# kongzhecn/OMG

Hardware: NVIDIA H100
Metric: 1024^2 images/sec @30 steps, 2 concepts (higher is better)
Workload: dtype f16

## Files before the change

### omg_b200/csrc/attn_relpos.cu

```cuda
#include <cuda_fp16.h>

#include <algorithm>
#include <math.h>
#include <string.h>

#include "../../include/omg_b200.h"
#include "host_common.h"
#include "ptx.cuh"
#include "wgmma.cuh"

namespace omg {

constexpr int RP_BQ = 128;
constexpr int RP_BKV = 64;
constexpr int RP_TROWS = 128;
constexpr int RP_STAGES = 3;
constexpr int RP_THREADS = 256;
constexpr float RP_LOG2E = 1.4426950408889634f;

template <int D>
struct RpLayout {
    static constexpr bool X = D > 64;
    static constexpr int Q64 = RP_BQ * 128;
    static constexpr int Q_BYTES = Q64 + (X ? RP_BQ * 32 : 0);
    static constexpr int K64 = RP_BKV * 128, K16 = RP_BKV * 32;
    static constexpr int STAGE = 2 * K64 + (X ? 2 * K16 : 0);
    static constexpr int T64 = RP_TROWS * 128, T16 = RP_TROWS * 32;
    static constexpr int T_BYTES = 2 * T64 + (X ? 2 * T16 : 0);
    static_assert(T_BYTES <= RP_STAGES * STAGE, "tables must fit the K/V ring");
    static constexpr int FIXED = 1024 + Q_BYTES + RP_STAGES * STAGE + 8 * (2 + 2 * RP_STAGES) + 4 * RP_BKV + 4 * RP_BQ;
};

struct alignas(64) RelposParams {
    CUtensorMap q64, q16, kv64, kv16;
    CUtensorMap th64, th16, tw64, tw16;
    const __half* qkv;
    const __half* kb;
    const __half* vb;
    __half* out;
    long long bs, out_bs;
    int ld, out_ld, out_col0;
    int q_col0, k_col0, v_col0;
    int H, W, Wh, Ww;
    int nwx, ntiles, byq, byk, nkb;
    int sh_stride, sw_stride;
    int has_pad;
    float scale_log2;
};

static inline int rp_bias_stride(int S) {
    int s = (S + 7) / 8 * 8;
    return s % 16 == 0 ? s + 8 : s;
}

template <int D>
__global__ void __launch_bounds__(RP_THREADS, 1) attn_relpos_kernel(const __grid_constant__ RelposParams p) {
    using Lt = RpLayout<D>;
    constexpr bool X = Lt::X;
    extern __shared__ uint8_t smem_raw[];
    uint8_t* smem = reinterpret_cast<uint8_t*>((reinterpret_cast<uintptr_t>(smem_raw) + 1023) & ~uintptr_t(1023));
    uint8_t* q_smem = smem;
    uint8_t* kv_smem = q_smem + Lt::Q_BYTES;
    uint64_t* q_full = reinterpret_cast<uint64_t*>(kv_smem + RP_STAGES * Lt::STAGE);
    uint64_t* t_full = q_full + 1;
    uint64_t* kv_full = q_full + 2;
    uint64_t* kv_empty = kv_full + RP_STAGES;
    int* kmap = reinterpret_cast<int*>(kv_empty + RP_STAGES);
    float* qkb = reinterpret_cast<float*>(kmap + RP_BKV);
    float* bias_h = qkb + RP_BQ;
    float* bias_w = bias_h + RP_BQ * p.sh_stride;

    const int warp = threadIdx.x >> 5, lane = threadIdx.x & 31;
    const int tile = blockIdx.x % p.ntiles, grp = blockIdx.x / p.ntiles;
    const int y0 = (grp / p.nwx) * p.Wh, x0 = (grp % p.nwx) * p.Ww;
    const int head = blockIdx.y, img = blockIdx.z;
    const int nq_box = p.Ww * p.byq, nk_box = p.Ww * p.byk;
    const int qc = p.q_col0 + head * D, kc = p.k_col0 + head * D, vc = p.v_col0 + head * D;
    const int qy_base = tile * p.byq;

    for (int i = threadIdx.x; i < (RP_BQ - nq_box) * 8; i += RP_THREADS)
        reinterpret_cast<uint4*>(q_smem + nq_box * 128)[i] = make_uint4(0, 0, 0, 0);
    if (X)
        for (int i = threadIdx.x; i < (RP_BQ - nq_box) * 2; i += RP_THREADS)
            reinterpret_cast<uint4*>(q_smem + Lt::Q64 + nq_box * 32)[i] = make_uint4(0, 0, 0, 0);
    if (threadIdx.x == 0) {
        tma_prefetch_desc(&p.q64);
        tma_prefetch_desc(&p.kv64);
        mbar_init(q_full, 1);
        mbar_init(t_full, 1);
        for (int i = 0; i < RP_STAGES; ++i) {
            mbar_init(&kv_full[i], 1);
            mbar_init(&kv_empty[i], 2);
        }
        fence_barrier_init();
    }
    if (threadIdx.x < RP_BKV) {
        const int kr = threadIdx.x;
        kmap[kr] = kr < nk_box ? ((kr / p.Ww) << 8) | (kr % p.Ww) : -1;
    }
    fence_proxy_async_smem();
    __syncthreads();
    griddep_launch_dependents();
    griddep_wait();
    if (threadIdx.x == 0) {
        mbar_arrive_expect_tx(q_full, nq_box * D * 2);
        tma_load_4d(q_smem, &p.q64, q_full, qc, x0, y0 + qy_base, img);
        if (X) tma_load_4d(q_smem + Lt::Q64, &p.q16, q_full, qc + 64, x0, y0 + qy_base, img);
        mbar_arrive_expect_tx(t_full, 2 * RP_TROWS * D * 2);
        tma_load_2d(kv_smem, &p.th64, t_full, 0, 0);
        tma_load_2d(kv_smem + Lt::T64, &p.tw64, t_full, 0, 0);
        if (X) {
            tma_load_2d(kv_smem + 2 * Lt::T64, &p.th16, t_full, 64, 0);
            tma_load_2d(kv_smem + 2 * Lt::T64 + Lt::T16, &p.tw16, t_full, 64, 0);
        }
    }
    if (p.has_pad && threadIdx.x < RP_BQ) {
        const int r = threadIdx.x;
        const int gy = y0 + qy_base + r / p.Ww, gx = x0 + r % p.Ww;
        float acc = 0.f;
        if (r < nq_box && gy < p.H && gx < p.W) {
            const __half* q = p.qkv + img * p.bs + (long long)(gy * p.W + gx) * p.ld + qc;
            const __half* kb = p.kb + head * D;
#pragma unroll 8
            for (int d = 0; d < D; ++d) acc = fmaf(__half2float(q[d]), __half2float(kb[d]), acc);
        }
        qkb[r] = acc * p.scale_log2;
    }

    const int wg = warp >> 2, wi = warp & 3;
    const int g = lane >> 2, c = lane & 3;
    const int row0 = wg * 64 + wi * 16 + g;
    const uint32_t q_addr = smem_u32(q_smem) + wg * (64 * 128);
    const uint32_t q16_addr = smem_u32(q_smem + Lt::Q64) + wg * (64 * 32);
    mbar_wait(q_full, 0);
    mbar_wait(t_full, 0);
#pragma unroll 1
    for (int t = 0; t < 2; ++t) {
        const int S = t ? p.Ww : p.Wh;
        float* bias = t ? bias_w : bias_h;
        const int stride = t ? p.sw_stride : p.sh_stride;
        const uint32_t t_addr = smem_u32(kv_smem) + t * Lt::T64;
        const uint32_t t16_addr = smem_u32(kv_smem) + 2 * Lt::T64 + t * Lt::T16;
        int qpos[2];
#pragma unroll
        for (int hh = 0; hh < 2; ++hh) {
            const int r = row0 + 8 * hh;
            qpos[hh] = t ? r % p.Ww : min(qy_base + r / p.Ww, p.Wh - 1);
        }
#pragma unroll 1
        for (int ch = 0; ch * 64 < 2 * S - 1; ++ch) {
            float acc[32];
#pragma unroll
            for (int i = 0; i < 32; ++i) acc[i] = 0.f;
            wgmma_fence();
#pragma unroll
            for (int k = 0; k < 4; ++k)
                wgmma_ss_n64(acc, gmma_desc_sw128(q_addr + k * 32, 1024, 16),
                             gmma_desc_sw128(t_addr + ch * 8192 + k * 32, 1024, 16), 1u);
            if (X) wgmma_ss_n64(acc, gmma_desc_sw32(q16_addr), gmma_desc_sw32(t16_addr + ch * 2048), 1u);
            wgmma_commit();
            wgmma_wait<0>();
            reg_fence(acc);
#pragma unroll
            for (int J = 0; J < 8; ++J)
#pragma unroll
                for (int hh = 0; hh < 2; ++hh)
#pragma unroll
                    for (int e = 0; e < 2; ++e) {
                        const int k = qpos[hh] + S - 1 - (ch * 64 + 8 * J + 2 * c + e);
                        if (k >= 0 && k < S) bias[(row0 + 8 * hh) * stride + k] = acc[4 * J + 2 * hh + e] * RP_LOG2E;
                    }
        }
    }
    __syncthreads();
    for (int st = 0; st < RP_STAGES; ++st) {
        uint8_t* sd = kv_smem + st * Lt::STAGE;
        for (int i = threadIdx.x; i < (RP_BKV - nk_box) * 8; i += RP_THREADS) {
            reinterpret_cast<uint4*>(sd + nk_box * 128)[i] = make_uint4(0, 0, 0, 0);
            reinterpret_cast<uint4*>(sd + Lt::K64 + nk_box * 128)[i] = make_uint4(0, 0, 0, 0);
        }
        if (X)
            for (int i = threadIdx.x; i < (RP_BKV - nk_box) * 2; i += RP_THREADS) {
                reinterpret_cast<uint4*>(sd + 2 * Lt::K64 + nk_box * 32)[i] = make_uint4(0, 0, 0, 0);
                reinterpret_cast<uint4*>(sd + 2 * Lt::K64 + Lt::K16 + nk_box * 32)[i] = make_uint4(0, 0, 0, 0);
            }
    }
    fence_proxy_async_smem();
    __syncthreads();

    auto load_kv = [&](int jb) {
        const int st = jb % RP_STAGES;
        mbar_wait(&kv_empty[st], ((jb / RP_STAGES) & 1) ^ 1);
        uint8_t* sd = kv_smem + st * Lt::STAGE;
        const int y = y0 + jb * p.byk;
        mbar_arrive_expect_tx(&kv_full[st], 2 * nk_box * D * 2);
        tma_load_4d(sd, &p.kv64, &kv_full[st], kc, x0, y, img);
        tma_load_4d(sd + Lt::K64, &p.kv64, &kv_full[st], vc, x0, y, img);
        if (X) {
            tma_load_4d(sd + 2 * Lt::K64, &p.kv16, &kv_full[st], kc + 64, x0, y, img);
            tma_load_4d(sd + 2 * Lt::K64 + Lt::K16, &p.kv16, &kv_full[st], vc + 64, x0, y, img);
        }
    };
    if (threadIdx.x == 0)
        for (int jb = 0; jb < RP_STAGES && jb < p.nkb; ++jb) load_kv(jb);

    const float* bh[2] = {bias_h + row0 * p.sh_stride, bias_h + (row0 + 8) * p.sh_stride};
    const float* bw[2] = {bias_w + row0 * p.sw_stride, bias_w + (row0 + 8) * p.sw_stride};
    const float qk[2] = {p.has_pad ? qkb[row0] : 0.f, p.has_pad ? qkb[row0 + 8] : 0.f};
    float o[32], o16[8];
#pragma unroll
    for (int i = 0; i < 32; ++i) o[i] = 0.f;
#pragma unroll
    for (int i = 0; i < 8; ++i) o16[i] = 0.f;
    float m[2] = {-INFINITY, -INFINITY}, l[2] = {0.f, 0.f}, lp[2] = {0.f, 0.f};
    for (int j = 0; j < p.nkb; ++j) {
        const int st = j % RP_STAGES;
        mbar_wait(&kv_full[st], (j / RP_STAGES) & 1);
        const uint32_t k_addr = smem_u32(kv_smem + st * Lt::STAGE);
        float s[32];
#pragma unroll
        for (int i = 0; i < 32; ++i) s[i] = 0.f;
        wgmma_fence();
#pragma unroll
        for (int k = 0; k < 4; ++k)
            wgmma_ss_n64(s, gmma_desc_sw128(q_addr + k * 32, 1024, 16), gmma_desc_sw128(k_addr + k * 32, 1024, 16), 1u);
        if (X) wgmma_ss_n64(s, gmma_desc_sw32(q16_addr), gmma_desc_sw32(k_addr + 2 * Lt::K64), 1u);
        wgmma_commit();
        if (threadIdx.x == 0 && j >= 1 && j - 1 + RP_STAGES < p.nkb) load_kv(j - 1 + RP_STAGES);
        __syncwarp();
        wgmma_wait<0>();
        reg_fence(s);
        uint32_t padbits = 0;
#pragma unroll
        for (int J = 0; J < 8; ++J)
#pragma unroll
            for (int e = 0; e < 2; ++e) {
                const int km = kmap[8 * J + 2 * c + e];
                const int ky = j * p.byk + (km >> 8), kx = km & 255;
                const bool valid = km >= 0 && ky < p.Wh;
                const bool pad = valid && (y0 + ky >= p.H || x0 + kx >= p.W);
                padbits |= (uint32_t)pad << (2 * J + e);
#pragma unroll
                for (int hh = 0; hh < 2; ++hh) {
                    float& v = s[4 * J + 2 * hh + e];
                    v = valid ? fmaf(v, p.scale_log2, bh[hh][ky] + bw[hh][kx] + (pad ? qk[hh] : 0.f)) : -INFINITY;
                }
            }
        float mx[2] = {-INFINITY, -INFINITY};
#pragma unroll
        for (int J = 0; J < 8; ++J)
#pragma unroll
            for (int hh = 0; hh < 2; ++hh) mx[hh] = fmaxf(mx[hh], fmaxf(s[4 * J + 2 * hh], s[4 * J + 2 * hh + 1]));
        float corr[2];
#pragma unroll
        for (int hh = 0; hh < 2; ++hh) {
            mx[hh] = fmaxf(mx[hh], __shfl_xor_sync(0xffffffffu, mx[hh], 1));
            mx[hh] = fmaxf(mx[hh], __shfl_xor_sync(0xffffffffu, mx[hh], 2));
            const float m_new = fmaxf(m[hh], mx[hh]);
            corr[hh] = fast_exp2(m[hh] - m_new);
            m[hh] = m_new;
            l[hh] *= corr[hh];
            lp[hh] *= corr[hh];
        }
#pragma unroll
        for (int J = 0; J < 8; ++J)
#pragma unroll
            for (int hh = 0; hh < 2; ++hh) {
                o[4 * J + 2 * hh] *= corr[hh];
                o[4 * J + 2 * hh + 1] *= corr[hh];
            }
#pragma unroll
        for (int J = 0; J < 2; ++J)
#pragma unroll
            for (int hh = 0; hh < 2; ++hh) {
                o16[4 * J + 2 * hh] *= corr[hh];
                o16[4 * J + 2 * hh + 1] *= corr[hh];
            }
        uint32_t pa[4][4];
#pragma unroll
        for (int kk = 0; kk < 4; ++kk)
#pragma unroll
            for (int t = 0; t < 4; ++t) {
                const int hh = t & 1, J = 2 * kk + (t >> 1), i0 = 4 * J + 2 * hh;
                const float p0 = fast_exp2(s[i0] - m[hh]);
                const float p1 = fast_exp2(s[i0 + 1] - m[hh]);
                l[hh] += p0 + p1;
                if (padbits >> (2 * J) & 1u) lp[hh] += p0;
                if (padbits >> (2 * J + 1) & 1u) lp[hh] += p1;
                pa[kk][t] = pack_half2(p0, p1);
            }
        const uint32_t v_addr = k_addr + Lt::K64;
        const uint32_t v16_addr = k_addr + 2 * Lt::K64 + Lt::K16;
        wgmma_fence();
#pragma unroll
        for (int kk = 0; kk < 4; ++kk) {
            wgmma_rs_n64_tb(o, pa[kk], gmma_desc_sw128(v_addr + kk * 2048, 1024, 1024), 1u);
            if (X) wgmma_rs_n16_tb(o16, pa[kk], gmma_desc_sw32(v16_addr + kk * 512), 1u);
        }
        wgmma_commit();
        wgmma_wait<0>();
        reg_fence(o);
        if constexpr (X) reg_fence(o16);
        if ((threadIdx.x & 127) == 0) mbar_arrive(&kv_empty[st]);
    }

#pragma unroll
    for (int hh = 0; hh < 2; ++hh) {
        l[hh] += __shfl_xor_sync(0xffffffffu, l[hh], 1);
        l[hh] += __shfl_xor_sync(0xffffffffu, l[hh], 2);
        lp[hh] += __shfl_xor_sync(0xffffffffu, lp[hh], 1);
        lp[hh] += __shfl_xor_sync(0xffffffffu, lp[hh], 2);
        const int r = row0 + 8 * hh;
        const int qy = qy_base + r / p.Ww, qx = r % p.Ww;
        const int gy = y0 + qy, gx = x0 + qx;
        if (r >= nq_box || qy >= p.Wh || gy >= p.H || gx >= p.W) continue;
        const float inv = 1.f / l[hh];
        __half* op = p.out + img * p.out_bs + (long long)(gy * p.W + gx) * p.out_ld + p.out_col0 + head * D + 2 * c;
        const __half* vb = p.has_pad ? p.vb + head * D + 2 * c : nullptr;
#pragma unroll
        for (int J = 0; J < 8; ++J) {
            float v0 = o[4 * J + 2 * hh], v1 = o[4 * J + 2 * hh + 1];
            if (vb) {
                v0 = fmaf(lp[hh], __half2float(vb[8 * J]), v0);
                v1 = fmaf(lp[hh], __half2float(vb[8 * J + 1]), v1);
            }
            *reinterpret_cast<__half2*>(op + 8 * J) = __floats2half2_rn(v0 * inv, v1 * inv);
        }
        if (X)
#pragma unroll
            for (int J = 0; J < 2; ++J) {
                float v0 = o16[4 * J + 2 * hh], v1 = o16[4 * J + 2 * hh + 1];
                if (vb) {
                    v0 = fmaf(lp[hh], __half2float(vb[64 + 8 * J]), v0);
                    v1 = fmaf(lp[hh], __half2float(vb[64 + 8 * J + 1]), v1);
                }
                *reinterpret_cast<__half2*>(op + 64 + 8 * J) = __floats2half2_rn(v0 * inv, v1 * inv);
            }
    }
}

static size_t rp_smem_bytes(int D, int Wh, int Ww) {
    const size_t fixed = D > 64 ? RpLayout<80>::FIXED : RpLayout<64>::FIXED;
    return fixed + (size_t)4 * RP_BQ * (rp_bias_stride(Wh) + rp_bias_stride(Ww));
}

template <int D>
static int launch_relpos(RelposParams& p, dim3 grid, size_t smem, cudaStream_t stream) {
    static bool configured = false;
    if (!configured) {
        OMG_CUDA(cudaFuncSetAttribute(attn_relpos_kernel<D>, cudaFuncAttributeMaxDynamicSharedMemorySize,
                                      (int)rp_smem_bytes(D, 64, 64)));
        configured = true;
    }
    OMG_CUDA(launch_pdl(attn_relpos_kernel<D>, grid, dim3(RP_THREADS), smem, stream, p));
    return check_launch(D > 64 ? "attn_relpos_kernel<80>" : "attn_relpos_kernel<64>");
}

}

using namespace omg;

static int relpos_impl(const omg_attn_relpos_desc* d, void* stream_) {
    static const char* who = "omg_attention_relpos";
    OMG_CHECK(d != nullptr, "%s: null descriptor", who);
    OMG_CHECK(d->head_dim == 64 || d->head_dim == 80, "%s: head_dim %d unsupported (SAM ViT-B/L use 64, ViT-H 80)", who,
              d->head_dim);
    OMG_CHECK(d->B >= 1 && d->H >= 1 && d->W >= 1 && d->heads >= 1, "%s: empty problem", who);
    OMG_CHECK(d->window >= 0 && d->window <= 64, "%s: window %d out of range [0, 64]", who, d->window);
    OMG_CHECK(d->window > 0 || (d->H <= 64 && d->W <= 64), "%s: global attention over a %d x %d grid (at most 64 x 64)",
              who, d->H, d->W);
    const int Wh = d->window ? d->window : d->H, Ww = d->window ? d->window : d->W;
    OMG_CHECK(d->rel_h_len == 2 * Wh - 1, "%s: rel_pos_h has %d rows, expected 2 * %d - 1 = %d (no interpolation)", who,
              d->rel_h_len, Wh, 2 * Wh - 1);
    OMG_CHECK(d->rel_w_len == 2 * Ww - 1, "%s: rel_pos_w has %d rows, expected 2 * %d - 1 = %d (no interpolation)", who,
              d->rel_w_len, Ww, 2 * Ww - 1);
    OMG_CHECK(d->qkv && d->out && d->rel_pos_h && d->rel_pos_w, "%s: null pointer", who);
    const bool pad = d->window > 0 && (d->H % d->window || d->W % d->window);
    OMG_CHECK(!pad || (d->k_bias && d->v_bias),
              "%s: a %d x %d grid in windows of %d is padded: k_bias and v_bias (the padded tokens' key and value) are "
              "required", who, d->H, d->W, d->window);
    OMG_CHECK(((uintptr_t)d->qkv & 15) == 0 && d->ld % 8 == 0 && d->bs % 8 == 0,
              "%s: qkv rows must be 16 B aligned (pointer, ld, bs)", who);
    OMG_CHECK(((uintptr_t)d->rel_pos_h & 15) == 0 && ((uintptr_t)d->rel_pos_w & 15) == 0,
              "%s: rel-pos tables must be 16 B aligned", who);
    OMG_CHECK(((uintptr_t)d->out & 15) == 0 && d->out_ld % 8 == 0 && d->out_col0 % 8 == 0 && d->out_bs % 8 == 0,
              "%s: output must be 16 B aligned per row", who);
    if (check_head_windows(who, d->heads, d->head_dim, {d->q_col0, d->k_col0, d->v_col0, d->out_col0},
                           {d->ld, d->ld, d->ld, d->out_ld}))
        return 1;

    const int D = d->head_dim;
    RelposParams p;
    memset(&p, 0, sizeof(p));
    const int byq = std::min(RP_BQ / Ww, Wh), byk = std::min(RP_BKV / Ww, Wh);
    const uint64_t dims[4] = {(uint64_t)d->ld, (uint64_t)d->W, (uint64_t)d->H, (uint64_t)d->B};
    const uint64_t strides[4] = {1, (uint64_t)d->ld, (uint64_t)d->ld * d->W, (uint64_t)d->bs};
    const uint32_t bq64[4] = {64, (uint32_t)Ww, (uint32_t)byq, 1}, bq16[4] = {16, (uint32_t)Ww, (uint32_t)byq, 1};
    const uint32_t bk64[4] = {64, (uint32_t)Ww, (uint32_t)byk, 1}, bk16[4] = {16, (uint32_t)Ww, (uint32_t)byk, 1};
    const auto F16 = CU_TENSOR_MAP_DATA_TYPE_FLOAT16;
    if (make_tmap(&p.q64, F16, d->qkv, 4, dims, strides, bq64, CU_TENSOR_MAP_SWIZZLE_128B)) return 1;
    if (make_tmap(&p.kv64, F16, d->qkv, 4, dims, strides, bk64, CU_TENSOR_MAP_SWIZZLE_128B)) return 1;
    const uint64_t th_dims[2] = {(uint64_t)D, (uint64_t)d->rel_h_len}, tw_dims[2] = {(uint64_t)D, (uint64_t)d->rel_w_len};
    const uint64_t t_str[2] = {1, (uint64_t)D};
    const uint32_t bt64[2] = {64, RP_TROWS}, bt16[2] = {16, RP_TROWS};
    if (make_tmap(&p.th64, F16, d->rel_pos_h, 2, th_dims, t_str, bt64, CU_TENSOR_MAP_SWIZZLE_128B)) return 1;
    if (make_tmap(&p.tw64, F16, d->rel_pos_w, 2, tw_dims, t_str, bt64, CU_TENSOR_MAP_SWIZZLE_128B)) return 1;
    if (D > 64) {
        if (make_tmap(&p.q16, F16, d->qkv, 4, dims, strides, bq16, CU_TENSOR_MAP_SWIZZLE_32B)) return 1;
        if (make_tmap(&p.kv16, F16, d->qkv, 4, dims, strides, bk16, CU_TENSOR_MAP_SWIZZLE_32B)) return 1;
        if (make_tmap(&p.th16, F16, d->rel_pos_h, 2, th_dims, t_str, bt16, CU_TENSOR_MAP_SWIZZLE_32B)) return 1;
        if (make_tmap(&p.tw16, F16, d->rel_pos_w, 2, tw_dims, t_str, bt16, CU_TENSOR_MAP_SWIZZLE_32B)) return 1;
    }
    p.qkv = static_cast<const __half*>(d->qkv);
    p.kb = static_cast<const __half*>(d->k_bias);
    p.vb = static_cast<const __half*>(d->v_bias);
    p.out = static_cast<__half*>(d->out);
    p.bs = d->bs;
    p.out_bs = d->out_bs;
    p.ld = d->ld;
    p.out_ld = d->out_ld;
    p.out_col0 = d->out_col0;
    p.q_col0 = d->q_col0;
    p.k_col0 = d->k_col0;
    p.v_col0 = d->v_col0;
    p.H = d->H;
    p.W = d->W;
    p.Wh = Wh;
    p.Ww = Ww;
    p.nwx = (d->W + Ww - 1) / Ww;
    p.byq = byq;
    p.byk = byk;
    p.ntiles = (Wh + byq - 1) / byq;
    p.nkb = (Wh + byk - 1) / byk;
    p.sh_stride = rp_bias_stride(Wh);
    p.sw_stride = rp_bias_stride(Ww);
    p.has_pad = pad;
    p.scale_log2 = d->scale * RP_LOG2E;
    const int nwy = (d->H + Wh - 1) / Wh;
    const dim3 grid(nwy * p.nwx * p.ntiles, d->heads, d->B);
    const size_t smem = rp_smem_bytes(D, Wh, Ww);
    cudaStream_t stream = reinterpret_cast<cudaStream_t>(stream_);
    return D > 64 ? launch_relpos<80>(p, grid, smem, stream) : launch_relpos<64>(p, grid, smem, stream);
}

extern "C" int omg_attention_relpos(const omg_attn_relpos_desc* d, void* stream_) {
    const int rc = relpos_impl(d, stream_);
    if (rc == 0 && ::omg::plan_recording()) {
        const omg_attn_relpos_desc c = *d;
        ::omg::plan_note([c](void* s) { return relpos_impl(&c, s); });
    }
    return rc;
}
```

### omg_b200/csrc/attn_tc.cu

```cuda
#include <cuda_fp16.h>

#include <algorithm>
#include <math.h>
#include <stdlib.h>
#include <string.h>

#include "../../include/omg_b200.h"
#include "host_common.h"
#include "ptx.cuh"
#include "wgmma.cuh"

namespace omg {

constexpr int ATT_BQ = 128;
constexpr int ATT_BKV = 64;
constexpr int ATT_D = 64;
constexpr int ATT_Q_BYTES = ATT_BQ * ATT_D * 2;
constexpr int ATT_K_BYTES = ATT_BKV * ATT_D * 2;
constexpr int ATT_KV_STAGES = 4;
constexpr int ATT_THREADS = 256;
constexpr int ATT_SMEM = 1024 + ATT_Q_BYTES + ATT_KV_STAGES * 2 * ATT_K_BYTES + 256;

struct alignas(64) AttnParams {
    CUtensorMap q_map, k_map, v_map;
    __half* out;
    int out_ld;
    long long out_bs;
    int n_q, n_kv, heads;
    int q_col0, k_col0, v_col0, out_col0;
    int n_items;
    int out_b[OMG_ATTN_MAX_ITEMS], q_b[OMG_ATTN_MAX_ITEMS], k_b[OMG_ATTN_MAX_ITEMS], v_b[OMG_ATTN_MAX_ITEMS];
    float scale_log2;
    float out_weight;
    int accumulate;
    int causal;
};

__global__ void __launch_bounds__(ATT_THREADS, 2) attn_tc_kernel(const __grid_constant__ AttnParams p) {
    extern __shared__ uint8_t smem_raw[];
    uint8_t* smem = reinterpret_cast<uint8_t*>((reinterpret_cast<uintptr_t>(smem_raw) + 1023) & ~uintptr_t(1023));
    uint8_t* q_smem = smem;
    uint8_t* kv_smem = q_smem + ATT_Q_BYTES;
    uint64_t* q_full = reinterpret_cast<uint64_t*>(kv_smem + ATT_KV_STAGES * 2 * ATT_K_BYTES);
    uint64_t* kv_full = q_full + 1;
    uint64_t* kv_empty = kv_full + ATT_KV_STAGES;

    const int warp = threadIdx.x >> 5;
    const int lane = threadIdx.x & 31;
    const int slab = blockIdx.x, head = blockIdx.y, item = blockIdx.z;
    const int nkv = (p.n_kv + ATT_BKV - 1) / ATT_BKV;

    const int kb = p.k_b[item], vb = p.v_b[item];
    auto load_kv = [&](int jb) {
        const int st = jb % ATT_KV_STAGES;
        mbar_wait(&kv_empty[st], ((jb / ATT_KV_STAGES) & 1) ^ 1);
        uint8_t* kd = kv_smem + st * 2 * ATT_K_BYTES;
        mbar_arrive_expect_tx(&kv_full[st], 2 * ATT_K_BYTES);
        tma_load_3d(kd, &p.k_map, &kv_full[st], p.k_col0 + head * ATT_D, jb * ATT_BKV, kb);
        tma_load_3d(kd + ATT_K_BYTES, &p.v_map, &kv_full[st], p.v_col0 + head * ATT_D, jb * ATT_BKV, vb);
    };
    if (threadIdx.x == 0) {
        tma_prefetch_desc(&p.q_map);
        tma_prefetch_desc(&p.k_map);
        tma_prefetch_desc(&p.v_map);
        mbar_init(q_full, 1);
        for (int i = 0; i < ATT_KV_STAGES; ++i) {
            mbar_init(&kv_full[i], 1);
            mbar_init(&kv_empty[i], 2);
        }
        fence_barrier_init();
    }
    __syncthreads();
    griddep_launch_dependents();
    griddep_wait();
    if (threadIdx.x == 0) {
        mbar_arrive_expect_tx(q_full, ATT_Q_BYTES);
        tma_load_3d(q_smem, &p.q_map, q_full, p.q_col0 + head * ATT_D, slab * ATT_BQ, p.q_b[item]);
        for (int jb = 0; jb < ATT_KV_STAGES && jb < nkv; ++jb) load_kv(jb);
    }

    const int wg = warp >> 2, wi = warp & 3;
    const int g = lane >> 2, c = lane & 3;
    const int qrow0 = slab * ATT_BQ + wg * 64 + wi * 16 + g;
    const uint32_t q_addr = smem_u32(q_smem) + wg * (64 * 128);
    float o[32];
#pragma unroll
    for (int i = 0; i < 32; ++i) o[i] = 0.f;
    float m[2] = {-INFINITY, -INFINITY}, l[2] = {0.f, 0.f};
    mbar_wait(q_full, 0);
    for (int j = 0; j < nkv; ++j) {
        const int st = j % ATT_KV_STAGES;
        mbar_wait(&kv_full[st], (j / ATT_KV_STAGES) & 1);
        const uint32_t k_addr = smem_u32(kv_smem + st * 2 * ATT_K_BYTES);
        float s[32];
#pragma unroll
        for (int i = 0; i < 32; ++i) s[i] = 0.f;
        wgmma_fence();
#pragma unroll
        for (int k = 0; k < ATT_D / 16; ++k)
            wgmma_ss_n64(s, gmma_desc_sw128(q_addr + k * 32, 1024, 16), gmma_desc_sw128(k_addr + k * 32, 1024, 16), 1u);
        wgmma_commit();
        if (threadIdx.x == 0 && j >= 1 && j - 1 + ATT_KV_STAGES < nkv) load_kv(j - 1 + ATT_KV_STAGES);
        __syncwarp();
        wgmma_wait<0>();
        reg_fence(s);
        const int key0 = j * ATT_BKV + 2 * c;
        if ((j + 1) * ATT_BKV > p.n_kv || p.causal) {
#pragma unroll
            for (int J = 0; J < 8; ++J)
#pragma unroll
                for (int h = 0; h < 2; ++h)
#pragma unroll
                    for (int e = 0; e < 2; ++e) {
                        const int key = key0 + 8 * J + e;
                        if (key >= p.n_kv || (p.causal && key > qrow0 + 8 * h)) s[4 * J + 2 * h + e] = -INFINITY;
                    }
        }
        float mx[2] = {-INFINITY, -INFINITY};
#pragma unroll
        for (int J = 0; J < 8; ++J)
#pragma unroll
            for (int h = 0; h < 2; ++h) mx[h] = fmaxf(mx[h], fmaxf(s[4 * J + 2 * h], s[4 * J + 2 * h + 1]));
        float corr[2];
#pragma unroll
        for (int h = 0; h < 2; ++h) {
            mx[h] = fmaxf(mx[h], __shfl_xor_sync(0xffffffffu, mx[h], 1));
            mx[h] = fmaxf(mx[h], __shfl_xor_sync(0xffffffffu, mx[h], 2));
            const float m_new = fmaxf(m[h], mx[h] * p.scale_log2);
            corr[h] = fast_exp2(m[h] - m_new);
            m[h] = m_new;
            l[h] *= corr[h];
        }
#pragma unroll
        for (int J = 0; J < 8; ++J)
#pragma unroll
            for (int h = 0; h < 2; ++h) {
                o[4 * J + 2 * h] *= corr[h];
                o[4 * J + 2 * h + 1] *= corr[h];
            }
        uint32_t pa[4][4];
#pragma unroll
        for (int kk = 0; kk < 4; ++kk)
#pragma unroll
            for (int t = 0; t < 4; ++t) {
                const int h = t & 1, i0 = 8 * kk + 4 * (t >> 1) + 2 * h;
                const float p0 = fast_exp2(fmaf(s[i0], p.scale_log2, -m[h]));
                const float p1 = fast_exp2(fmaf(s[i0 + 1], p.scale_log2, -m[h]));
                l[h] += p0 + p1;
                pa[kk][t] = pack_half2(p0, p1);
            }
        const uint32_t v_addr = k_addr + ATT_K_BYTES;
        wgmma_fence();
#pragma unroll
        for (int kk = 0; kk < 4; ++kk)
            wgmma_rs_n64_tb(o, pa[kk], gmma_desc_sw128(v_addr + kk * 2048, 1024, 1024), 1u);
        wgmma_commit();
        wgmma_wait<0>();
        reg_fence(o);
        if ((threadIdx.x & 127) == 0) mbar_arrive(&kv_empty[st]);
    }

#pragma unroll
    for (int h = 0; h < 2; ++h) {
        l[h] += __shfl_xor_sync(0xffffffffu, l[h], 1);
        l[h] += __shfl_xor_sync(0xffffffffu, l[h], 2);
        const int qrow = qrow0 + 8 * h;
        if (qrow < p.n_q) {
            const float inv = p.out_weight / l[h];
            __half* op = p.out + (long long)p.out_b[item] * p.out_bs + (long long)qrow * p.out_ld + p.out_col0 +
                         head * ATT_D + 2 * c;
#pragma unroll
            for (int J = 0; J < 8; ++J) {
                float v0 = o[4 * J + 2 * h] * inv, v1 = o[4 * J + 2 * h + 1] * inv;
                __half2* dst = reinterpret_cast<__half2*>(op + 8 * J);
                if (p.accumulate) {
                    const float2 f = __half22float2(*dst);
                    v0 += f.x;
                    v1 += f.y;
                }
                *dst = __floats2half2_rn(v0, v1);
            }
        }
    }
}

static int make_attn_map(CUtensorMap* m, const void* ptr, int cols, int ld, int tokens, long long bs, int nb,
                         uint32_t box_rows) {
    const uint64_t dims[3] = {(uint64_t)cols, (uint64_t)tokens, (uint64_t)nb};
    const uint64_t strides[3] = {1, (uint64_t)ld, (uint64_t)bs};
    const uint32_t box[3] = {64, box_rows, 1};
    return make_tmap(m, CU_TENSOR_MAP_DATA_TYPE_FLOAT16, ptr, 3, dims, strides, box, CU_TENSOR_MAP_SWIZZLE_128B);
}

}

using namespace omg;

static int attention_impl(const omg_attn_desc* d, void* stream_) {
    cudaStream_t stream = reinterpret_cast<cudaStream_t>(stream_);
    OMG_CHECK(d != nullptr, "omg_attention: null descriptor");
    OMG_CHECK(d->head_dim == 64, "omg_attention: head_dim %d unsupported (SDXL uses 64)", d->head_dim);
    OMG_CHECK(d->n_items >= 1 && d->n_items <= OMG_ATTN_MAX_ITEMS, "omg_attention: n_items=%d out of range",
              d->n_items);
    OMG_CHECK(d->n_q >= 1 && d->n_kv >= 1 && d->heads >= 1, "omg_attention: empty problem");
    OMG_CHECK(d->q && d->k && d->v && d->out, "omg_attention: null pointer");
    OMG_CHECK(d->out_ld % 8 == 0 && d->out_col0 % 8 == 0 && d->out_bs % 8 == 0,
              "omg_attention: output must be 16 B aligned per row");
    if (check_head_windows("omg_attention", d->heads, d->head_dim, {d->q_col0, d->k_col0, d->v_col0, d->out_col0},
                           {d->q_ld, d->k_ld, d->v_ld, d->out_ld}))
        return 1;
    OMG_CHECK(!d->causal || (d->n_kv <= 128 && d->n_q <= 128), "omg_attention: causal masking is available for sequences of <= 128 tokens");
    static bool configured = false;
    if (!configured) {
        OMG_CUDA(cudaFuncSetAttribute(attn_tc_kernel, cudaFuncAttributeMaxDynamicSharedMemorySize, ATT_SMEM));
        configured = true;
    }
    AttnParams p;
    memset(&p, 0, sizeof(p));
    int max_qb = 0, max_kb = 0, max_vb = 0;
    for (int i = 0; i < d->n_items; ++i) {
        p.out_b[i] = d->out_b[i];
        p.q_b[i] = d->q_b[i];
        p.k_b[i] = d->k_b[i];
        p.v_b[i] = d->v_b[i];
        max_qb = d->q_b[i] > max_qb ? d->q_b[i] : max_qb;
        max_kb = d->k_b[i] > max_kb ? d->k_b[i] : max_kb;
        max_vb = d->v_b[i] > max_vb ? d->v_b[i] : max_vb;
        OMG_CHECK(d->out_b[i] >= 0 && d->q_b[i] >= 0 && d->k_b[i] >= 0 && d->v_b[i] >= 0,
                  "omg_attention: negative batch index in item %d", i);
    }
    const int cols = d->heads * 64;
    if (make_attn_map(&p.q_map, d->q, d->q_col0 + cols, d->q_ld, d->n_q, d->q_bs, max_qb + 1, ATT_BQ)) return 1;
    if (make_attn_map(&p.k_map, d->k, d->k_col0 + cols, d->k_ld, d->n_kv, d->k_bs, max_kb + 1, ATT_BKV)) return 1;
    if (make_attn_map(&p.v_map, d->v, d->v_col0 + cols, d->v_ld, d->n_kv, d->v_bs, max_vb + 1, ATT_BKV)) return 1;
    p.out = static_cast<__half*>(d->out);
    p.out_ld = d->out_ld;
    p.out_bs = d->out_bs;
    p.n_q = d->n_q;
    p.n_kv = d->n_kv;
    p.heads = d->heads;
    p.q_col0 = d->q_col0;
    p.k_col0 = d->k_col0;
    p.v_col0 = d->v_col0;
    p.out_col0 = d->out_col0;
    p.n_items = d->n_items;
    p.scale_log2 = d->scale * 1.4426950408889634f;
    p.out_weight = d->out_weight;
    p.accumulate = d->accumulate;
    p.causal = d->causal;
    dim3 grid((d->n_q + ATT_BQ - 1) / ATT_BQ, d->heads, d->n_items);
    OMG_CUDA(launch_pdl(attn_tc_kernel, grid, dim3(ATT_THREADS), ATT_SMEM, stream, p));
    return check_launch("attn_tc_kernel");
}

extern "C" int omg_attention(const omg_attn_desc* d, void* stream_) {
    const int rc = attention_impl(d, stream_);
    if (rc == 0 && ::omg::plan_recording()) {
        const omg_attn_desc c = *d;
        ::omg::plan_note([c](void* s) { return attention_impl(&c, s); });
    }
    return rc;
}
```

### omg_b200/csrc/gemm_tc.cu

```cuda
#include <cuda_fp16.h>
#include <stdlib.h>
#include <string.h>

#include <algorithm>
#include <type_traits>

#include "../../include/omg_b200.h"
#include "elem.cuh"
#include "host_common.h"
#include "ptx.cuh"
#include "wgmma.cuh"

namespace omg {

constexpr int BM = 128;
constexpr int BK = 64;
constexpr int GEMM_THREADS = 384;

struct SegDev {
    int a_map, dx, dy, a_c0, k_blocks, b_k0, b_map;
};

struct alignas(64) GemmParams {
    CUtensorMap a_maps[OMG_MAX_A];
    CUtensorMap b_maps[2];
    SegDev segs[OMG_MAX_SEGS];
    int n_segs;
    int m_tiles, n_tiles;
    int tw, th, tiles_w, tiles_h;
    int img_w, img_h, img_b;
    int N, N_out;
    void* out;
    long long out_sw, out_sh, out_sb;
    const void* bias;
    const void* rowvec;
    int rowvec_ld;
    const void* residual;
    int residual_ld;
    int act_silu;
    float* stats_out;
    const float* stats_in;
    int stats_parts;
    long long stats_rows;
    float ln_inv_dim, ln_eps;
    const float* col_c1;
    const float* col_c2;
    int n_col_groups;
    long long col_group_end[8];
    int w_group_rows;
    const float* residual_f32;
    long long residual_f32_ld;
    float* out_f32;
    long long out_f32_ld;
    float4* col_stats;
    int cs_rb0, cs_rb_total;
};

template <int BN, int MT, bool CS>
struct GemmCfg {
    static constexpr int WN = BN > 256 ? BN / 2 : BN;
    static constexpr int NW = BN / WN;
    static constexpr int ACC = MT * BN / 2;
    static constexpr int A_BYTES = MT * BM * BK * 2;
    static constexpr int B_BYTES = BN * BK * 2;
    static constexpr int STAGE_BYTES = A_BYTES + B_BYTES;
    static constexpr int VEC_BYTES = 2 * MT * BN * 4;
    static constexpr int CS_BYTES = CS ? 8 * MT * BN * 8 : 0;
    static constexpr int BARS_BYTES = 256;
    static constexpr int BUDGET = 227 * 1024 - 1024  - VEC_BYTES - CS_BYTES - BARS_BYTES;
    static constexpr int STAGES_RAW = BUDGET / STAGE_BYTES;
    static constexpr int STAGES = STAGES_RAW > 8 ? 8 : STAGES_RAW;
    static constexpr int SMEM_BYTES = 1024 + STAGES * STAGE_BYTES + VEC_BYTES + CS_BYTES + BARS_BYTES;
    static_assert(STAGES >= 2, "shared memory budget");
};

__device__ __forceinline__ float gelu_exact(float x) { return 0.5f * x * (1.0f + erff(x * 0.70710678118654752f)); }

template <typename T, int WN>
__device__ __forceinline__ void wgmma_ss(float* d, uint64_t da, uint64_t db) {
    if constexpr (std::is_same_v<T, __nv_bfloat16>) {
        if constexpr (WN == 64) wgmma_ss_n64_bf16(*reinterpret_cast<float(*)[32]>(d), da, db, 1u);
        else if constexpr (WN == 128) wgmma_ss_n128_bf16(*reinterpret_cast<float(*)[64]>(d), da, db, 1u);
        else if constexpr (WN == 160) wgmma_ss_n160_bf16(*reinterpret_cast<float(*)[80]>(d), da, db, 1u);
        else wgmma_ss_n256_bf16(*reinterpret_cast<float(*)[128]>(d), da, db, 1u);
    } else {
        if constexpr (WN == 64) wgmma_ss_n64(*reinterpret_cast<float(*)[32]>(d), da, db, 1u);
        else if constexpr (WN == 128) wgmma_ss_n128(*reinterpret_cast<float(*)[64]>(d), da, db, 1u);
        else if constexpr (WN == 160) wgmma_ss_n160(*reinterpret_cast<float(*)[80]>(d), da, db, 1u);
        else wgmma_ss_n256(*reinterpret_cast<float(*)[128]>(d), da, db, 1u);
    }
}

template <typename T, int BN, int EPI, int MT, int FEAT>
__global__ void __launch_bounds__(GEMM_THREADS, 1) gemm_tc_kernel(const __grid_constant__ GemmParams p) {
    using T2 = pair_t<T>;
    constexpr bool kStats = FEAT >= 1, kExtra = FEAT >= 2;
    static_assert(EPI != OMG_EPI_GEGLU || (BN <= 256 && MT == 1), "GEGLU runs on single 128-row tiles");
    using Cfg = GemmCfg<BN, MT, kStats>;
    constexpr int STAGES = Cfg::STAGES;
    constexpr int NJ = BN / 8;
    extern __shared__ __align__(1024) uint8_t smem_raw[];
    uint8_t* smem = reinterpret_cast<uint8_t*>((reinterpret_cast<uintptr_t>(smem_raw) + 1023) & ~uintptr_t(1023));
    float* s_bias = reinterpret_cast<float*>(smem + STAGES * Cfg::STAGE_BYTES);
    float* s_c1 = s_bias + MT * BN;
    float4* s_cs = reinterpret_cast<float4*>(s_c1 + MT * BN);
    uint64_t* full_bar = reinterpret_cast<uint64_t*>(reinterpret_cast<uint8_t*>(s_cs) + Cfg::CS_BYTES);
    uint64_t* empty_bar = full_bar + STAGES;

    const int warp = threadIdx.x >> 5;
    const int lane = threadIdx.x & 31;
    const int total_tiles = ((p.m_tiles + MT - 1) / MT) * p.n_tiles;
    const int tiles_per_img = p.tiles_w * p.tiles_h;

    if (warp == 8 && lane == 0) {
        for (int i = 0; i < OMG_MAX_A; ++i) tma_prefetch_desc(&p.a_maps[i]);
        tma_prefetch_desc(&p.b_maps[0]);
        tma_prefetch_desc(&p.b_maps[1]);
        for (int i = 0; i < STAGES; ++i) {
            mbar_init(&full_bar[i], 1);
            mbar_init(&empty_bar[i], 2);
        }
        fence_barrier_init();
    }
    __syncthreads();
    griddep_launch_dependents();
    griddep_wait();

    if (warp >= 8) {
        asm volatile("setmaxnreg.dec.sync.aligned.u32 40;");
        if (warp == 8 && lane == 0) {
            int stage = 0;
            uint32_t phase = 0;
            for (int tile = blockIdx.x; tile < total_tiles; tile += gridDim.x) {
                const int m_tile = (tile / p.n_tiles) * MT, n_tile = tile % p.n_tiles;
                const int b = m_tile / tiles_per_img;
                const int rem = m_tile % tiles_per_img;
                const int h0 = (rem / p.tiles_w) * p.th, w0 = (rem % p.tiles_w) * p.tw;
                const int b1 = (m_tile + 1) / tiles_per_img, rem1 = (m_tile + 1) % tiles_per_img;
                const int h1 = (rem1 / p.tiles_w) * p.th, w1 = (rem1 % p.tiles_w) * p.tw;
                int n0 = n_tile * BN;
                if (p.w_group_rows > 0) {
                    const long long tile_pix0 = ((long long)b * p.img_h + h0) * p.img_w + w0;
                    for (int g2 = 0; g2 + 1 < p.n_col_groups; ++g2)
                        if (tile_pix0 >= p.col_group_end[g2]) n0 += p.w_group_rows;
                }
                for (int s = 0; s < p.n_segs; ++s) {
                    const SegDev sg = p.segs[s];
                    for (int kb = 0; kb < sg.k_blocks; ++kb) {
                        mbar_wait(&empty_bar[stage], phase ^ 1);
                        uint8_t* a_dst = smem + stage * Cfg::STAGE_BYTES;
                        uint8_t* b_dst = a_dst + Cfg::A_BYTES;
                        mbar_arrive_expect_tx(&full_bar[stage], Cfg::STAGE_BYTES);
                        tma_load_4d(a_dst, &p.a_maps[sg.a_map], &full_bar[stage], sg.a_c0 + kb * BK, w0 + sg.dx, h0 + sg.dy, b);
                        if constexpr (MT == 2)
                            tma_load_4d(a_dst + BM * BK * 2, &p.a_maps[sg.a_map], &full_bar[stage], sg.a_c0 + kb * BK,
                                        w1 + sg.dx, h1 + sg.dy, b1);
#pragma unroll
                        for (int nw = 0; nw < Cfg::NW; ++nw)
                            tma_load_2d(b_dst + nw * Cfg::WN * BK * 2, &p.b_maps[sg.b_map], &full_bar[stage],
                                        sg.b_k0 + kb * BK, n0 + nw * Cfg::WN);
                        if (++stage == STAGES) {
                            stage = 0;
                            phase ^= 1;
                        }
                    }
                }
            }
        }
        return;
    }

    asm volatile("setmaxnreg.inc.sync.aligned.u32 232;");
    const int wg = warp >> 2;
    const int wi = warp & 3;
    const int g = lane >> 2, c = lane & 3;
    const int ctid = threadIdx.x;
    int stage = 0;
    uint32_t phase = 0;
    float acc[Cfg::ACC];

    for (int tile = blockIdx.x; tile < total_tiles; tile += gridDim.x) {
        const int unit_m = (tile / p.n_tiles) * MT, n_tile = tile % p.n_tiles;
        const int n0 = n_tile * BN;
        const bool ln = p.stats_in != nullptr;

        named_bar_sync(1, 256);
        for (int sub = 0; sub < MT; ++sub) {
            const int mt = unit_m + sub;
            const int b = mt / tiles_per_img, rem = mt % tiles_per_img;
            size_t cg = 0;
            if (ln && p.n_col_groups > 1) {
                const long long tile_pix0 = ((long long)b * p.img_h + (rem / p.tiles_w) * p.th) * p.img_w + (rem % p.tiles_w) * p.tw;
                for (int g2 = 0; g2 + 1 < p.n_col_groups; ++g2)
                    if (tile_pix0 >= p.col_group_end[g2]) cg = g2 + 1;
                cg *= (size_t)p.N;
            }
            for (int j = ctid; j < BN; j += 256) {
                float v = 0.f, c1 = 0.f;
                const int n = n0 + j;
                if (n < p.N) {
                    if (ln) {
                        v = p.col_c2[cg + n];
                        c1 = p.col_c1[cg + n];
                    } else {
                        if (p.bias) v += to_f32(static_cast<const T*>(p.bias)[n]);
                        if (p.rowvec && b < p.img_b) v += to_f32(static_cast<const T*>(p.rowvec)[(size_t)b * p.rowvec_ld + n]);
                    }
                }
                s_bias[sub * BN + j] = v;
                s_c1[sub * BN + j] = c1;
            }
        }
        named_bar_sync(1, 256);

#pragma unroll
        for (int i = 0; i < Cfg::ACC; ++i) acc[i] = 0.f;
        int prev_stage = -1;
        for (int s = 0; s < p.n_segs; ++s) {
            const int kbs = p.segs[s].k_blocks;
            for (int kb = 0; kb < kbs; ++kb) {
                mbar_wait(&full_bar[stage], phase);
                const uint32_t a_addr = smem_u32(smem + stage * Cfg::STAGE_BYTES) + (uint32_t)(wg * MT) * (64 * BK * 2);
                const uint32_t b_addr = smem_u32(smem + stage * Cfg::STAGE_BYTES + Cfg::A_BYTES);
                wgmma_fence();
#pragma unroll
                for (int k = 0; k < BK / 16; ++k) {
#pragma unroll
                    for (int i = 0; i < MT; ++i) {
                        const uint64_t a_desc = gmma_desc_sw128(a_addr + i * (64 * BK * 2) + k * 32, 1024, 16);
#pragma unroll
                        for (int nw = 0; nw < Cfg::NW; ++nw) {
                            const uint64_t b_desc = gmma_desc_sw128(b_addr + nw * (Cfg::WN * BK * 2) + k * 32, 1024, 16);
                            wgmma_ss<T, Cfg::WN>(acc + i * (BN / 2) + nw * (Cfg::WN / 2), a_desc, b_desc);
                        }
                    }
                }
                wgmma_commit();
                wgmma_wait<1>();
                if (prev_stage >= 0 && (ctid & 127) == 0) mbar_arrive(&empty_bar[prev_stage]);
                prev_stage = stage;
                if (++stage == STAGES) {
                    stage = 0;
                    phase ^= 1;
                }
            }
        }
        wgmma_wait<0>();
        reg_fence(acc);
        if ((ctid & 127) == 0) mbar_arrive(&empty_bar[prev_stage]);

#pragma unroll
        for (int i = 0; i < MT; ++i) {
            const int blk = wg * MT + i;
            const int sub = blk >> 1;
            const int m_tile = unit_m + sub;
            const int b = m_tile / tiles_per_img;
            const int rem = m_tile % tiles_per_img;
            const int h0 = (rem / p.tiles_w) * p.th, w0 = (rem % p.tiles_w) * p.tw;
            const float* sb = s_bias + sub * BN;
            const float* sc = s_c1 + sub * BN;
            float* a = acc + i * (BN / 2);
            float row_sum[2] = {0.f, 0.f}, row_sq[2] = {0.f, 0.f};
            bool valid[2];
            size_t pix[2];
            T* orow[2];
            float ln_a[2] = {1.f, 1.f}, ln_k[2] = {0.f, 0.f};
#pragma unroll
            for (int h = 0; h < 2; ++h) {
                const int et = (blk & 1) * 64 + wi * 16 + g + 8 * h;
                const int ph = h0 + et / p.tw, pw = w0 + et % p.tw;
                valid[h] = (ph < p.img_h) && (pw < p.img_w) && (b < p.img_b);
                pix[h] = ((size_t)b * p.img_h + ph) * p.img_w + pw;
                orow[h] = static_cast<T*>(p.out) + (long long)b * p.out_sb + (long long)ph * p.out_sh + (long long)pw * p.out_sw;
                if (ln && valid[h]) {
                    float sa = 0.f, sq = 0.f;
                    for (int t = 0; t < p.stats_parts; ++t) {
                        const float2 st = __ldg(reinterpret_cast<const float2*>(p.stats_in) + (size_t)t * p.stats_rows + pix[h]);
                        sa += st.x;
                        sq += st.y;
                    }
                    const float mu = sa * p.ln_inv_dim;
                    ln_a[h] = rsqrtf(fmaxf(sq * p.ln_inv_dim - mu * mu, 0.f) + p.ln_eps);
                    ln_k[h] = -ln_a[h] * mu;
                }
            }
            float4* cs_slot = s_cs + (size_t)(blk * 4 + wi) * (BN / 2);
#pragma unroll
            for (int J = 0; J < NJ; ++J) {
                const int col = 8 * J + 2 * c;
                const int n = n0 + col;
                float x[2][2];
#pragma unroll
                for (int h = 0; h < 2; ++h)
#pragma unroll
                    for (int e = 0; e < 2; ++e) {
                        const float v = a[4 * J + 2 * h + e];
                        x[h][e] = ln ? fmaf(ln_a[h], v, fmaf(ln_k[h], sc[col + e], sb[col + e])) : v + sb[col + e];
                    }
                if constexpr (EPI == OMG_EPI_GEGLU) {
#pragma unroll
                    for (int h = 0; h < 2; ++h) {
                        const float o = x[h][0] * gelu_exact(x[h][1]);
                        const float o_nb = __shfl_down_sync(0xffffffffu, o, 1);
                        if ((c & 1) == 0 && valid[h] && n < p.N)
                            *reinterpret_cast<T2*>(orow[h] + (n >> 1)) = from_f32x2<T>(o, o_nb);
                    }
                } else {
                    if constexpr (kExtra) {
#pragma unroll
                        for (int h = 0; h < 2; ++h)
#pragma unroll
                            for (int e = 0; e < 2; ++e) {
                                float v = x[h][e];
                                if (p.act_silu == 1) {
                                    v = v / (1.0f + __expf(-v));
                                } else if (p.act_silu == 2) {
                                    v = v / (1.0f + __expf(-1.702f * v));
                                } else if (p.act_silu == 3) {
                                    v = gelu_exact(v);
                                } else if (p.act_silu == 4) {
                                    const float u = 0.7978845608028654f * fmaf(0.044715f * v * v, v, v);
                                    v = 0.5f * v * (2.0f - __fdividef(2.0f, 1.0f + __expf(2.0f * u)));
                                } else if (p.act_silu == 5) {
                                    v = fmaxf(v, 0.f);
                                }
                                x[h][e] = v;
                            }
                    }
                    float4 cs = make_float4(0.f, 0.f, 0.f, 0.f);
#pragma unroll
                    for (int h = 0; h < 2; ++h) {
                        const bool ok = valid[h] && n < p.N;
                        if (ok && p.residual != nullptr) {
                            const float2 r = to_f32x2(*reinterpret_cast<const T2*>(static_cast<const T*>(p.residual) + pix[h] * (size_t)p.residual_ld + n));
                            x[h][0] += r.x;
                            x[h][1] += r.y;
                        }
                        if constexpr (kExtra) {
                            if (ok && p.residual_f32 != nullptr) {
                                const float2 r = *reinterpret_cast<const float2*>(p.residual_f32 + pix[h] * (size_t)p.residual_f32_ld + n);
                                x[h][0] += r.x;
                                x[h][1] += r.y;
                            }
                            if (ok && p.out_f32 != nullptr)
                                *reinterpret_cast<float2*>(p.out_f32 + pix[h] * (size_t)p.out_f32_ld + n) = make_float2(x[h][0], x[h][1]);
                        }
                        if (ok) {
                            row_sum[h] += x[h][0] + x[h][1];
                            row_sq[h] = fmaf(x[h][0], x[h][0], fmaf(x[h][1], x[h][1], row_sq[h]));
                        }
                        const T2 o = from_f32x2<T>(x[h][0], x[h][1]);
                        if (ok) *reinterpret_cast<T2*>(orow[h] + n) = o;
                        if constexpr (kStats) {
                            const float2 f = valid[h] ? to_f32x2(o) : make_float2(0.f, 0.f);
                            cs.x += f.x;
                            cs.y = fmaf(f.x, f.x, cs.y);
                            cs.z += f.y;
                            cs.w = fmaf(f.y, f.y, cs.w);
                        }
                    }
                    if constexpr (kStats) {
                        if (p.col_stats != nullptr) {
#pragma unroll
                            for (int off = 4; off < 32; off <<= 1) {
                                cs.x += __shfl_xor_sync(0xffffffffu, cs.x, off);
                                cs.y += __shfl_xor_sync(0xffffffffu, cs.y, off);
                                cs.z += __shfl_xor_sync(0xffffffffu, cs.z, off);
                                cs.w += __shfl_xor_sync(0xffffffffu, cs.w, off);
                            }
                            if (g == 0) cs_slot[4 * J + c] = cs;
                        }
                    }
                }
            }
            if constexpr (EPI != OMG_EPI_GEGLU) {
                if (p.stats_out != nullptr) {
                    float2* so = reinterpret_cast<float2*>(p.stats_out);
                    constexpr int PLANES = BN > 256 ? 4 : 2;
#pragma unroll
                    for (int h = 0; h < 2; ++h) {
                        float s = row_sum[h], q = row_sq[h];
                        s += __shfl_xor_sync(0xffffffffu, s, 1);
                        q += __shfl_xor_sync(0xffffffffu, q, 1);
                        s += __shfl_xor_sync(0xffffffffu, s, 2);
                        q += __shfl_xor_sync(0xffffffffu, q, 2);
                        if (c == 0 && valid[h]) {
                            so[(size_t)(n_tile * PLANES) * p.stats_rows + pix[h]] = make_float2(s, q);
                            for (int t = 1; t < PLANES; ++t) so[(size_t)(n_tile * PLANES + t) * p.stats_rows + pix[h]] = make_float2(0.f, 0.f);
                        }
                    }
                }
            }
            if constexpr (EPI != OMG_EPI_GEGLU && kStats) {
                if (p.col_stats != nullptr) {
                    named_bar_sync(2 + wg * 2 + (wi >> 1), 64);
                    const int q = (blk & 1) * 2 + (wi >> 1);
                    const float4* s0 = s_cs + (size_t)(blk * 4 + (wi & 2)) * (BN / 2);
                    const float4* s1 = s0 + BN / 2;
                    if (b < p.img_b) {
                        const size_t rb = (size_t)b * p.cs_rb_total + p.cs_rb0 + (size_t)rem * 4 + q;
                        for (int cp = (wi & 1) * 32 + lane; cp < BN / 2; cp += 64) {
                            const int col = n0 + 2 * cp;
                            if (col < p.N) {
                                const float4 u = s0[cp], w = s1[cp];
                                p.col_stats[(rb * p.N + col) >> 1] = make_float4(u.x + w.x, u.y + w.y, u.z + w.z, u.w + w.w);
                            }
                        }
                    }
                }
            }
        }
    }
}

static int view_to_tmap(CUtensorMap* m, const omg_view4& v, CUtensorMapDataType dt, uint32_t box_c, uint32_t box_w,
                        uint32_t box_h, CUtensorMapSwizzle sw) {
    const uint64_t dims[4] = {(uint64_t)v.C, (uint64_t)v.W, (uint64_t)v.H, (uint64_t)v.B};
    const uint64_t strides[4] = {1, (uint64_t)v.sw, (uint64_t)v.sh, (uint64_t)v.sb};
    const uint32_t box[4] = {box_c, box_w, box_h, 1};
    return make_tmap(m, dt, v.ptr, 4, dims, strides, box, sw);
}

template <typename T, int BN, int EPI, int MT, int FEAT>
static int launch_gemm_f(const GemmParams& p, cudaStream_t stream) {
    using Cfg = GemmCfg<BN, MT, (FEAT >= 1)>;
    static bool configured = false;
    static int num_sms = 0;
    if (!configured) {
        OMG_CUDA(cudaFuncSetAttribute(gemm_tc_kernel<T, BN, EPI, MT, FEAT>, cudaFuncAttributeMaxDynamicSharedMemorySize,
                                      Cfg::SMEM_BYTES));
        int dev = 0;
        OMG_CUDA(cudaGetDevice(&dev));
        OMG_CUDA(cudaDeviceGetAttribute(&num_sms, cudaDevAttrMultiProcessorCount, dev));
        configured = true;
    }
    const int units = ((p.m_tiles + MT - 1) / MT) * p.n_tiles;
    const int grid = std::min(units, num_sms);
    OMG_CUDA(launch_pdl(gemm_tc_kernel<T, BN, EPI, MT, FEAT>, dim3(grid), dim3(GEMM_THREADS), Cfg::SMEM_BYTES, stream, p));
    return check_launch("gemm_tc_kernel");
}

template <int BN, int EPI, int MT = 1>
static int launch_gemm(const GemmParams& p, cudaStream_t stream) {
    if constexpr (EPI == OMG_EPI_GEGLU) {
        return launch_gemm_f<__half, BN, EPI, MT, 0>(p, stream);
    } else {
        if (p.act_silu != 0 || p.residual_f32 != nullptr || p.out_f32 != nullptr) return launch_gemm_f<__half, BN, EPI, MT, 2>(p, stream);
        if (p.col_stats != nullptr) return launch_gemm_f<__half, BN, EPI, MT, 1>(p, stream);
        return launch_gemm_f<__half, BN, EPI, MT, 0>(p, stream);
    }
}

constexpr int PLAN_SMS = 132;
constexpr double TILE_OVERHEAD = 48.0;
static double tile_time(long tiles, double cols) {
    return (double)((tiles + PLAN_SMS - 1) / PLAN_SMS) * (cols + TILE_OVERHEAD);
}

static bool use_tall_tiles(long m_tiles, long n_tiles, long k_blocks) {
    if (m_tiles < 2 || k_blocks < 16) return false;
    return tile_time(((m_tiles + 1) / 2) * n_tiles, 320.0) < tile_time(m_tiles * n_tiles, 160.0);
}

constexpr long K_PLAN_LONG = 1000;
static int pick_block_n(int N, int epilogue, long m_tiles, long k_plan, long k_blocks, bool* prefer_tall) {
    if (prefer_tall) *prefer_tall = false;
    if (epilogue == OMG_EPI_GEGLU) return 256;
    const int cands[5] = {256, 160, 128, 64, 160};
    int best = 256;
    double best_t = 1e30;
    for (int i = 0; i < 5; ++i) {
        const bool tall = i == 4;
        if (tall && (k_plan < 16 || m_tiles < 2)) continue;
        const long nt = (N + cands[i] - 1) / cands[i];
        const long mt = tall ? (m_tiles + 1) / 2 : m_tiles;
        const double t = tile_time(nt * mt, tall ? 2.0 * cands[i] : cands[i]);
        if (t < best_t - 1e-9) {
            best_t = t;
            best = cands[i];
            if (prefer_tall) *prefer_tall = tall && k_blocks >= 16;
        }
    }
    return best;
}

}

using namespace omg;

extern "C" int omg_gemm_plan(int N, int epilogue, int W, int H, int B, int* block_n, int* n_tiles) {
    OMG_CHECK(N >= 8 && W >= 1 && H >= 1 && B >= 1, "omg_gemm_plan: bad arguments");
    int tw = 128;
    while (tw / 2 >= W && tw > 1) tw /= 2;
    const int th = 128 / tw;
    const long m_tiles = (long)((W + tw - 1) / tw) * ((H + th - 1) / th) * B;
    const int bn = pick_block_n(N, epilogue, m_tiles, K_PLAN_LONG, 0, nullptr);
    if (block_n) *block_n = bn;
    if (n_tiles) *n_tiles = 2 * ((N + bn - 1) / bn);
    return 0;
}

extern "C" int omg_gemm_colstats_blocks(int W, int H) {
    if (W < 1 || H < 1) return 0;
    int tw = 128;
    while (tw / 2 >= W && tw > 1) tw /= 2;
    const int th = 128 / tw;
    return ((W + tw - 1) / tw) * ((H + th - 1) / th) * 4;
}

static int gemm_impl(const omg_gemm_desc* d, void* stream_) {
    cudaStream_t stream = reinterpret_cast<cudaStream_t>(stream_);
    OMG_CHECK(d != nullptr, "omg_gemm: null descriptor");
    OMG_CHECK(d->n_a >= 1 && d->n_a <= OMG_MAX_A, "omg_gemm: n_a=%d out of range", d->n_a);
    OMG_CHECK(d->n_segs >= 1 && d->n_segs <= OMG_MAX_SEGS, "omg_gemm: n_segs=%d out of range", d->n_segs);
    OMG_CHECK(d->w && d->d.ptr, "omg_gemm: null weight/output pointer");
    OMG_CHECK(d->N >= 8 && d->N % 8 == 0, "omg_gemm: N=%d must be a positive multiple of 8", d->N);
    OMG_CHECK(d->Ktot % 8 == 0, "omg_gemm: Ktot=%d must be a multiple of 8", d->Ktot);
    OMG_CHECK(d->dtype == OMG_DTYPE_F16 || d->dtype == OMG_DTYPE_BF16, "omg_gemm: dtype=%d unsupported (0 fp16, 1 bf16)",
              d->dtype);
    const bool bf16 = d->dtype == OMG_DTYPE_BF16;
    if (bf16) {
        OMG_CHECK(d->epilogue == OMG_EPI_NONE, "omg_gemm: bf16 supports only OMG_EPI_NONE (epilogue %d)", d->epilogue);
        OMG_CHECK(!d->rowvec, "omg_gemm: bf16 does not support rowvec");
        OMG_CHECK(!d->w2, "omg_gemm: bf16 does not support a second weight matrix (w2)");
        OMG_CHECK(d->w_group_planes == 0, "omg_gemm: bf16 does not support weight planes");
        OMG_CHECK(!d->row_stats_in, "omg_gemm: bf16 does not support the folded LayerNorm");
        OMG_CHECK(!d->row_stats_out, "omg_gemm: bf16 does not support row statistics");
        OMG_CHECK(!d->col_stats_out, "omg_gemm: bf16 does not support column statistics");
        OMG_CHECK(!d->residual_f32 && !d->out_f32, "omg_gemm: bf16 does not support fp32 twins");
    }
    const CUtensorMapDataType tdt = bf16 ? CU_TENSOR_MAP_DATA_TYPE_BFLOAT16 : CU_TENSOR_MAP_DATA_TYPE_FLOAT16;
    const bool geglu = d->epilogue == OMG_EPI_GEGLU;
    const bool silu = d->epilogue == OMG_EPI_SILU;
    const int act = silu ? 1 : (d->epilogue == OMG_EPI_QUICK_GELU ? 2 : (d->epilogue == OMG_EPI_GELU ? 3 : (d->epilogue == OMG_EPI_GELU_TANH ? 4 :
                    (d->epilogue == OMG_EPI_RELU ? 5 : 0))));
    OMG_CHECK(d->epilogue == OMG_EPI_NONE || geglu || act, "omg_gemm: unknown epilogue %d", d->epilogue);
    const int N_out = geglu ? d->N / 2 : d->N;
    OMG_CHECK(d->d.C == N_out, "omg_gemm: output view has %d channels, expected %d", d->d.C, N_out);
    OMG_CHECK(!geglu || (d->N % 64 == 0 && !d->residual && !d->rowvec),
              "omg_gemm: GEGLU needs N %% 64 == 0 and no residual/rowvec");
    OMG_CHECK(!d->residual || (N_out % 32 == 0 && d->residual_ld % 8 == 0),
              "omg_gemm: residual needs N %% 32 == 0 and ld %% 8 == 0");

    GemmParams p;
    memset(&p, 0, sizeof(p));
    const int W = d->d.W, H = d->d.H, B = d->d.B;
    OMG_CHECK(W >= 1 && H >= 1 && B >= 1, "omg_gemm: empty output grid");
    int tw = 128;
    while (tw / 2 >= W && tw > 1) tw /= 2;
    const int th = 128 / tw;
    p.tw = tw;
    p.th = th;
    p.tiles_w = (W + tw - 1) / tw;
    p.tiles_h = (H + th - 1) / th;
    p.img_w = W;
    p.img_h = H;
    p.img_b = B;
    p.m_tiles = p.tiles_w * p.tiles_h * B;
    p.N = d->N;
    p.N_out = N_out;
    bool prefer_tall = false;
    const long k_blocks_hint = (long)(d->Ktot + (d->w2 ? d->K2tot : 0)) / 64;
    int bn = d->block_n ? d->block_n
                        : pick_block_n(d->N, d->epilogue, p.m_tiles, d->row_stats_out ? K_PLAN_LONG : k_blocks_hint,
                                       k_blocks_hint, &prefer_tall);
    OMG_CHECK(bn == 64 || bn == 128 || bn == 160 || bn == 256 || bn == 320, "omg_gemm: block_n=%d unsupported", bn);
    OMG_CHECK(bn != 320 || (!geglu && d->N % 320 == 0), "omg_gemm: block_n=320 needs N %% 320 == 0 and no GEGLU");
    OMG_CHECK(d->cta_pair == 0 || d->cta_pair == 1 || d->cta_pair == 3, "omg_gemm: cta_pair=%d unsupported (0, 1 or 3)",
              d->cta_pair);
    if (geglu) bn = 256;
    p.n_tiles = (d->N + bn - 1) / bn;
    p.bias = d->bias;
    p.rowvec = d->rowvec;
    p.rowvec_ld = d->rowvec_ld;
    p.residual = d->residual;
    p.residual_ld = d->residual_ld;
    p.act_silu = act;
    p.stats_out = static_cast<float*>(d->row_stats_out);
    p.stats_in = static_cast<const float*>(d->row_stats_in);
    p.stats_parts = d->row_stats_parts;
    p.stats_rows = d->row_stats_stride > 0 ? d->row_stats_stride : (long long)W * H * B;
    p.ln_inv_dim = d->ln_dim > 0 ? 1.0f / (float)d->ln_dim : 0.f;
    p.ln_eps = d->ln_eps;
    p.col_c1 = static_cast<const float*>(d->col_c1);
    p.col_c2 = static_cast<const float*>(d->col_c2);
    p.n_col_groups = d->n_col_groups > 0 ? d->n_col_groups : 1;
    p.w_group_rows = d->w_group_planes > 0 ? d->N : 0;
    OMG_CHECK(d->w_group_planes == 0 || d->w_group_planes == p.n_col_groups, "omg_gemm: w_group_planes must equal n_col_groups");
    OMG_CHECK(p.n_col_groups <= 8, "omg_gemm: at most 8 column-vector row groups");
    OMG_CHECK(d->w_group_planes == 0 || !d->w2, "omg_gemm: weight planes do not extend to the second weight matrix (w2)");
    const long long img_pix = (long long)W * H;
    for (int i = 0; i < 8; ++i) {
        p.col_group_end[i] = d->col_group_end[i];
        if (i + 1 >= p.n_col_groups) continue;
        if (H > 1)
            OMG_CHECK(d->col_group_end[i] % img_pix == 0,
                      "omg_gemm: row-group boundary %lld is inside an image of the %d x %d output grid (boundaries are "
                      "multiples of %lld pixels)", (long long)d->col_group_end[i], W, H, img_pix);
        else
            OMG_CHECK(d->col_group_end[i] % 128 == 0, "omg_gemm: row-group boundary %lld is not a multiple of the 128-row tile",
                      (long long)d->col_group_end[i]);
    }
    OMG_CHECK(!p.stats_in || (p.col_c1 && p.col_c2 && d->ln_dim > 0 && d->row_stats_parts >= 1 && !d->rowvec),
              "omg_gemm: folded LayerNorm needs col_c1, col_c2, ln_dim, row_stats_parts and no rowvec");
    OMG_CHECK(!p.stats_out || !geglu, "omg_gemm: row statistics cannot be emitted by the GEGLU epilogue");
    p.residual_f32 = static_cast<const float*>(d->residual_f32);
    p.residual_f32_ld = d->residual_f32_ld;
    p.out_f32 = static_cast<float*>(d->out_f32);
    p.out_f32_ld = d->out_f32_ld;
    OMG_CHECK((!p.residual_f32 && !p.out_f32) || (!geglu && d->N % 32 == 0 && !(d->residual && d->residual_f32)),
              "omg_gemm: fp32 residual / output twins need a non-GEGLU epilogue, N %% 32 == 0, and replace the fp16 residual");
    OMG_CHECK((!p.residual_f32 || d->residual_f32_ld % 4 == 0) && (!p.out_f32 || d->out_f32_ld % 4 == 0),
              "omg_gemm: fp32 twin row strides must be multiples of 4");
    OMG_CHECK((!p.residual_f32 && !p.out_f32) || (d->d.sw == d->d.C && d->d.sh == (int64_t)d->d.sw * W && d->d.sb == d->d.sh * H),
              "omg_gemm: fp32 twins need a contiguous output view (rows are indexed by pixel)");
    p.col_stats = static_cast<float4*>(d->col_stats_out);
    p.cs_rb0 = d->col_stats_rb0;
    p.cs_rb_total = d->col_stats_rb_total;
    OMG_CHECK(!p.col_stats || (!geglu && d->N % 32 == 0 && d->col_stats_rb0 >= 0 &&
                               d->col_stats_rb0 + p.tiles_w * p.tiles_h * 4 <= d->col_stats_rb_total),
              "omg_gemm: column statistics need a non-GEGLU epilogue, N %% 32 == 0 and rb0 + blocks <= rb_total");
    OMG_CHECK((!p.stats_out && !p.stats_in) || (d->d.sw == d->d.C && d->d.sh == (int64_t)d->d.sw * W && d->d.sb == d->d.sh * H),
              "omg_gemm: row statistics need a contiguous output view");

    for (int i = 0; i < d->n_a; ++i) {
        OMG_CHECK(d->a[i].ptr != nullptr, "omg_gemm: A view %d is null", i);
        if (view_to_tmap(&p.a_maps[i], d->a[i], tdt, BK, tw, th, CU_TENSOR_MAP_SWIZZLE_128B)) return 1;
    }
    for (int i = d->n_a; i < OMG_MAX_A; ++i) p.a_maps[i] = p.a_maps[0];
    {
        const uint64_t planes = d->w_group_planes > 0 ? (uint64_t)d->w_group_planes : 1;
        const uint64_t dims[2] = {(uint64_t)d->Ktot, (uint64_t)d->N * planes};
        const uint64_t strides[2] = {1, (uint64_t)d->Ktot};
        const uint32_t box[2] = {BK, (uint32_t)(bn > 256 ? bn / 2 : bn)};
        if (make_tmap(&p.b_maps[0], tdt, d->w, 2, dims, strides, box, CU_TENSOR_MAP_SWIZZLE_128B)) return 1;
        p.b_maps[1] = p.b_maps[0];
    }
    if (d->w2 != nullptr) {
        OMG_CHECK(d->K2tot >= 8 && d->K2tot % 8 == 0, "omg_gemm: K2tot=%d must be a positive multiple of 8", d->K2tot);
        const uint64_t dims[2] = {(uint64_t)d->K2tot, (uint64_t)d->N};
        const uint64_t strides[2] = {1, (uint64_t)d->K2tot};
        const uint32_t box[2] = {BK, (uint32_t)(bn > 256 ? bn / 2 : bn)};
        if (make_tmap(&p.b_maps[1], tdt, d->w2, 2, dims, strides, box, CU_TENSOR_MAP_SWIZZLE_128B)) return 1;
    }
    OMG_CHECK(d->d.sw % 2 == 0 && d->d.sh % 2 == 0 && d->d.sb % 2 == 0 && (reinterpret_cast<uintptr_t>(d->d.ptr) & 3) == 0,
              "omg_gemm: output view must be 4 B aligned per pixel");
    p.out = const_cast<void*>(d->d.ptr);
    p.out_sw = d->d.sw;
    p.out_sh = d->d.sh;
    p.out_sb = d->d.sb;

    p.n_segs = d->n_segs;
    for (int s = 0; s < d->n_segs; ++s) {
        const omg_seg& sg = d->segs[s];
        OMG_CHECK(sg.a_idx >= 0 && sg.a_idx < d->n_a, "omg_gemm: segment %d references A view %d", s, sg.a_idx);
        OMG_CHECK(sg.k_len > 0 && sg.a_c0 >= 0 && sg.b_k0 >= 0 && sg.a_c0 + sg.k_len <= d->a[sg.a_idx].C,
                  "omg_gemm: segment %d has a bad K range", s);
        OMG_CHECK(sg.b_idx == 0 || (sg.b_idx == 1 && d->w2 != nullptr), "omg_gemm: segment %d has a bad b_idx", s);
        const int ktot_s = sg.b_idx ? d->K2tot : d->Ktot;
        OMG_CHECK(sg.b_k0 + sg.k_len <= ktot_s, "omg_gemm: segment %d exceeds weight K (%d + %d > %d)", s, sg.b_k0,
                  sg.k_len, ktot_s);
        OMG_CHECK(sg.k_len % BK == 0 || sg.a_c0 + sg.k_len == d->a[sg.a_idx].C,
                  "omg_gemm: segment %d: K tail must end at the A view's last channel", s);
        p.segs[s] = SegDev{sg.a_idx, sg.dx, sg.dy, sg.a_c0, (sg.k_len + BK - 1) / BK, sg.b_k0, sg.b_idx};
    }

    long k_blocks = 0;
    for (int i = 0; i < p.n_segs; ++i) k_blocks += p.segs[i].k_blocks;
    bool pair_ok = true;
    for (int i = 0; i + 1 < p.n_col_groups; ++i)
        pair_ok = pair_ok && (H > 1 ? (p.col_group_end[i] / img_pix * p.tiles_w * p.tiles_h) % 2 == 0
                                    : p.col_group_end[i] % 256 == 0);
    const bool tall = bn == 160 && !geglu && pair_ok &&
                      (d->cta_pair == 3 ||
                       (d->cta_pair == 0 && (prefer_tall || use_tall_tiles(p.m_tiles, p.n_tiles, k_blocks))));
    if (bf16) {
        if (tall) return launch_gemm_f<__nv_bfloat16, 160, OMG_EPI_NONE, 2, 0>(p, stream);
        switch (bn) {
            case 64: return launch_gemm_f<__nv_bfloat16, 64, OMG_EPI_NONE, 1, 0>(p, stream);
            case 128: return launch_gemm_f<__nv_bfloat16, 128, OMG_EPI_NONE, 1, 0>(p, stream);
            case 160: return launch_gemm_f<__nv_bfloat16, 160, OMG_EPI_NONE, 1, 0>(p, stream);
            case 320: return launch_gemm_f<__nv_bfloat16, 320, OMG_EPI_NONE, 1, 0>(p, stream);
            default: return launch_gemm_f<__nv_bfloat16, 256, OMG_EPI_NONE, 1, 0>(p, stream);
        }
    }
    if (bn == 320) return launch_gemm<320, OMG_EPI_NONE>(p, stream);
    if (tall) return launch_gemm<160, OMG_EPI_NONE, 2>(p, stream);
    if (geglu) return launch_gemm<256, OMG_EPI_GEGLU>(p, stream);
    switch (bn) {
        case 64: return launch_gemm<64, OMG_EPI_NONE>(p, stream);
        case 128: return launch_gemm<128, OMG_EPI_NONE>(p, stream);
        case 160: return launch_gemm<160, OMG_EPI_NONE>(p, stream);
        default: return launch_gemm<256, OMG_EPI_NONE>(p, stream);
    }
}

extern "C" int omg_gemm(const omg_gemm_desc* d, void* stream_) {
    const int rc = gemm_impl(d, stream_);
    if (rc == 0 && ::omg::plan_recording()) {
        const omg_gemm_desc c = *d;
        ::omg::plan_note([c](void* s) { return gemm_impl(&c, s); });
    }
    return rc;
}
```

### omg_b200/csrc/ptx.cuh

```cuda
#pragma once
#include <cuda.h>
#include <cuda_fp16.h>
#include <cuda_runtime.h>
#include <stdint.h>
#include <stdio.h>

namespace omg {

__device__ __forceinline__ uint32_t smem_u32(const void* p) {
    return static_cast<uint32_t>(__cvta_generic_to_shared(p));
}

__device__ __forceinline__ uint32_t lane_id() { return threadIdx.x & 31; }

__device__ __forceinline__ bool elect_one() {
    uint32_t pred;
    asm volatile(
        "{\n\t.reg .pred p;\n\t"
        "elect.sync _|p, 0xffffffff;\n\t"
        "selp.u32 %0, 1, 0, p;\n\t}\n"
        : "=r"(pred));
    return pred != 0;
}

__device__ __forceinline__ void griddep_launch_dependents() { asm volatile("griddepcontrol.launch_dependents;" ::: "memory"); }
__device__ __forceinline__ void griddep_wait() { asm volatile("griddepcontrol.wait;" ::: "memory"); }

__device__ __forceinline__ void mbar_init(uint64_t* bar, uint32_t count) {
    asm volatile("mbarrier.init.shared::cta.b64 [%0], %1;" ::"r"(smem_u32(bar)), "r"(count));
}
__device__ __forceinline__ void fence_barrier_init() {
    asm volatile("fence.mbarrier_init.release.cluster;" ::: "memory");
}
__device__ __forceinline__ void fence_proxy_async_smem() {
    asm volatile("fence.proxy.async.shared::cta;" ::: "memory");
}
__device__ __forceinline__ void mbar_arrive_expect_tx(uint64_t* bar, uint32_t bytes) {
    asm volatile("mbarrier.arrive.expect_tx.shared::cta.b64 _, [%0], %1;" ::"r"(smem_u32(bar)), "r"(bytes)
                 : "memory");
}
__device__ __forceinline__ void mbar_arrive(uint64_t* bar) {
    asm volatile("mbarrier.arrive.shared::cta.b64 _, [%0];" ::"r"(smem_u32(bar)) : "memory");
}
__device__ __forceinline__ bool mbar_try_wait(uint64_t* bar, uint32_t parity) {
    uint32_t ok;
    asm volatile(
        "{\n\t.reg .pred p;\n\t"
        "mbarrier.try_wait.parity.shared::cta.b64 p, [%1], %2;\n\t"
        "selp.u32 %0, 1, 0, p;\n\t}\n"
        : "=r"(ok)
        : "r"(smem_u32(bar)), "r"(parity)
        : "memory");
    return ok != 0;
}
#ifndef OMG_MBAR_TIMEOUT_CYCLES
#define OMG_MBAR_TIMEOUT_CYCLES (4000000000LL)
#endif
#ifndef OMG_MBAR_SUSPEND_NS
#define OMG_MBAR_SUSPEND_NS 20000
#endif
__device__ __forceinline__ bool mbar_try_wait_long(uint64_t* bar, uint32_t parity) {
    uint32_t ok;
    asm volatile(
        "{\n\t.reg .pred p;\n\t"
        "mbarrier.try_wait.parity.shared::cta.b64 p, [%1], %2, %3;\n\t"
        "selp.u32 %0, 1, 0, p;\n\t}\n"
        : "=r"(ok)
        : "r"(smem_u32(bar)), "r"(parity), "r"((uint32_t)OMG_MBAR_SUSPEND_NS)
        : "memory");
    return ok != 0;
}
__device__ __forceinline__ void mbar_wait(uint64_t* bar, uint32_t parity) {
    if (mbar_try_wait(bar, parity)) return;
    const long long t0 = clock64();
    uint32_t spins = 0;
    while (!mbar_try_wait_long(bar, parity)) {
        if ((++spins & 0x3FF) == 0 && clock64() - t0 > OMG_MBAR_TIMEOUT_CYCLES) {
            printf("omg: mbarrier timeout block=(%d,%d,%d) thread=%d bar=%u parity=%u\n", (int)blockIdx.x,
                   (int)blockIdx.y, (int)blockIdx.z, (int)threadIdx.x, smem_u32(bar), parity);
            __trap();
        }
    }
}

__device__ __forceinline__ float fast_exp2(float x) {
    float y;
    asm("ex2.approx.ftz.f32 %0, %1;" : "=f"(y) : "f"(x));
    return y;
}

__device__ __forceinline__ void tma_prefetch_desc(const CUtensorMap* m) {
    asm volatile("prefetch.tensormap [%0];" ::"l"(reinterpret_cast<uint64_t>(m)) : "memory");
}
__device__ __forceinline__ void tma_load_2d(void* smem_dst, const CUtensorMap* m, uint64_t* bar, int c0, int c1) {
    asm volatile(
        "cp.async.bulk.tensor.2d.shared::cluster.global.mbarrier::complete_tx::bytes [%0], [%1, {%3, %4}], [%2];"
        ::"r"(smem_u32(smem_dst)), "l"(reinterpret_cast<uint64_t>(m)), "r"(smem_u32(bar)), "r"(c0), "r"(c1)
        : "memory");
}
__device__ __forceinline__ void tma_load_3d(void* smem_dst, const CUtensorMap* m, uint64_t* bar, int c0, int c1,
                                            int c2) {
    asm volatile(
        "cp.async.bulk.tensor.3d.shared::cluster.global.mbarrier::complete_tx::bytes [%0], [%1, {%3, %4, %5}], [%2];"
        ::"r"(smem_u32(smem_dst)), "l"(reinterpret_cast<uint64_t>(m)), "r"(smem_u32(bar)), "r"(c0), "r"(c1), "r"(c2)
        : "memory");
}
__device__ __forceinline__ void tma_load_4d(void* smem_dst, const CUtensorMap* m, uint64_t* bar, int c0, int c1,
                                            int c2, int c3) {
    asm volatile(
        "cp.async.bulk.tensor.4d.shared::cluster.global.mbarrier::complete_tx::bytes [%0], [%1, {%3, %4, %5, %6}], "
        "[%2];"
        ::"r"(smem_u32(smem_dst)), "l"(reinterpret_cast<uint64_t>(m)), "r"(smem_u32(bar)), "r"(c0), "r"(c1), "r"(c2),
        "r"(c3)
        : "memory");
}
__device__ __forceinline__ void tma_store_3d(const CUtensorMap* m, const void* smem_src, int c0, int c1, int c2) {
    asm volatile("cp.async.bulk.tensor.3d.global.shared::cta.bulk_group [%0, {%2, %3, %4}], [%1];" ::"l"(
                     reinterpret_cast<uint64_t>(m)),
                 "r"(smem_u32(smem_src)), "r"(c0), "r"(c1), "r"(c2)
                 : "memory");
}
__device__ __forceinline__ void tma_store_4d(const CUtensorMap* m, const void* smem_src, int c0, int c1, int c2,
                                             int c3) {
    asm volatile("cp.async.bulk.tensor.4d.global.shared::cta.bulk_group [%0, {%2, %3, %4, %5}], [%1];" ::"l"(
                     reinterpret_cast<uint64_t>(m)),
                 "r"(smem_u32(smem_src)), "r"(c0), "r"(c1), "r"(c2), "r"(c3)
                 : "memory");
}
__device__ __forceinline__ void tma_store_commit() { asm volatile("cp.async.bulk.commit_group;" ::: "memory"); }
template <int N>
__device__ __forceinline__ void tma_store_wait_read() {
    asm volatile("cp.async.bulk.wait_group.read %0;" ::"n"(N) : "memory");
}
template <int N>
__device__ __forceinline__ void tma_store_wait_all() {
    asm volatile("cp.async.bulk.wait_group %0;" ::"n"(N) : "memory");
}

__device__ __forceinline__ uint64_t gmma_desc_sw128(uint32_t smem_addr, uint32_t sbo_bytes, uint32_t lbo_bytes) {
    uint64_t d = 0;
    d |= static_cast<uint64_t>((smem_addr & 0x3FFFF) >> 4);
    d |= static_cast<uint64_t>((lbo_bytes >> 4) & 0x3FFF) << 16;
    d |= static_cast<uint64_t>((sbo_bytes >> 4) & 0x3FFF) << 32;
    d |= static_cast<uint64_t>(1) << 62;
    return d;
}
__device__ __forceinline__ uint64_t gmma_desc_sw32(uint32_t smem_addr) {
    uint64_t d = 0;
    d |= static_cast<uint64_t>((smem_addr & 0x3FFFF) >> 4);
    d |= static_cast<uint64_t>(256 >> 4) << 16;
    d |= static_cast<uint64_t>(256 >> 4) << 32;
    d |= static_cast<uint64_t>(3) << 62;
    return d;
}
__device__ __forceinline__ void wgmma_fence() { asm volatile("wgmma.fence.sync.aligned;" ::: "memory"); }
__device__ __forceinline__ void wgmma_commit() { asm volatile("wgmma.commit_group.sync.aligned;" ::: "memory"); }
template <int N>
__device__ __forceinline__ void wgmma_wait() {
    asm volatile("wgmma.wait_group.sync.aligned %0;" ::"n"(N) : "memory");
}
template <int N>
__device__ __forceinline__ void reg_fence(float (&r)[N]) {
#pragma unroll
    for (int i = 0; i < N; ++i) asm volatile("" : "+f"(r[i])::"memory");
}
__device__ __forceinline__ void named_bar_sync(int id, int count) {
    asm volatile("bar.sync %0, %1;" ::"r"(id), "r"(count) : "memory");
}

__device__ __forceinline__ void st_shared_v4(uint32_t addr, uint32_t a, uint32_t b, uint32_t c, uint32_t d) {
    asm volatile("st.shared.v4.b32 [%0], {%1, %2, %3, %4};" ::"r"(addr), "r"(a), "r"(b), "r"(c), "r"(d) : "memory");
}

__device__ __forceinline__ uint32_t pack_half2(float a, float b) {
    __half2 h = __floats2half2_rn(a, b);
    return *reinterpret_cast<uint32_t*>(&h);
}

}
```

Baseline: 0.1891.

## Split GEMM tiles into per-warpgroup units with ping-pong mainloop turns

The GEMM kernel now has each of its two consumer warpgroups own a full 128-row by UN-column unit, alternating mainloop turns through turn barriers. One group's epilogue can then overlap the other's tensor-core work, and the tall two-M-tile variant and n256 instructions are removed. Mbarrier waits across the attention and GEMM kernels switch to an inlined wait variant to avoid call overhead. The trade-off is a narrower N per warpgroup, so B tiles are reloaded more often, and the epilogue plus stats layout gets more complex.

```diff
diff --git a/omg_b200/csrc/attn_relpos.cu b/omg_b200/csrc/attn_relpos.cu
--- a/omg_b200/csrc/attn_relpos.cu
+++ b/omg_b200/csrc/attn_relpos.cu
@@ -132,8 +132,8 @@
     const int row0 = wg * 64 + wi * 16 + g;
     const uint32_t q_addr = smem_u32(q_smem) + wg * (64 * 128);
     const uint32_t q16_addr = smem_u32(q_smem + Lt::Q64) + wg * (64 * 32);
-    mbar_wait(q_full, 0);
-    mbar_wait(t_full, 0);
+    mbar_wait_nocall(q_full, 0);
+    mbar_wait_nocall(t_full, 0);
 #pragma unroll 1
     for (int t = 0; t < 2; ++t) {
         const int S = t ? p.Ww : p.Wh;
@@ -190,7 +190,7 @@
 
     auto load_kv = [&](int jb) {
         const int st = jb % RP_STAGES;
-        mbar_wait(&kv_empty[st], ((jb / RP_STAGES) & 1) ^ 1);
+        mbar_wait_nocall(&kv_empty[st], ((jb / RP_STAGES) & 1) ^ 1);
         uint8_t* sd = kv_smem + st * Lt::STAGE;
         const int y = y0 + jb * p.byk;
         mbar_arrive_expect_tx(&kv_full[st], 2 * nk_box * D * 2);
@@ -215,7 +215,7 @@
     float m[2] = {-INFINITY, -INFINITY}, l[2] = {0.f, 0.f}, lp[2] = {0.f, 0.f};
     for (int j = 0; j < p.nkb; ++j) {
         const int st = j % RP_STAGES;
-        mbar_wait(&kv_full[st], (j / RP_STAGES) & 1);
+        mbar_wait_nocall(&kv_full[st], (j / RP_STAGES) & 1);
         const uint32_t k_addr = smem_u32(kv_smem + st * Lt::STAGE);
         float s[32];
 #pragma unroll
diff --git a/omg_b200/csrc/attn_tc.cu b/omg_b200/csrc/attn_tc.cu
--- a/omg_b200/csrc/attn_tc.cu
+++ b/omg_b200/csrc/attn_tc.cu
@@ -53,7 +53,7 @@
     const int kb = p.k_b[item], vb = p.v_b[item];
     auto load_kv = [&](int jb) {
         const int st = jb % ATT_KV_STAGES;
-        mbar_wait(&kv_empty[st], ((jb / ATT_KV_STAGES) & 1) ^ 1);
+        mbar_wait_nocall(&kv_empty[st], ((jb / ATT_KV_STAGES) & 1) ^ 1);
         uint8_t* kd = kv_smem + st * 2 * ATT_K_BYTES;
         mbar_arrive_expect_tx(&kv_full[st], 2 * ATT_K_BYTES);
         tma_load_3d(kd, &p.k_map, &kv_full[st], p.k_col0 + head * ATT_D, jb * ATT_BKV, kb);
@@ -87,10 +87,10 @@
 #pragma unroll
     for (int i = 0; i < 32; ++i) o[i] = 0.f;
     float m[2] = {-INFINITY, -INFINITY}, l[2] = {0.f, 0.f};
-    mbar_wait(q_full, 0);
+    mbar_wait_nocall(q_full, 0);
     for (int j = 0; j < nkv; ++j) {
         const int st = j % ATT_KV_STAGES;
-        mbar_wait(&kv_full[st], (j / ATT_KV_STAGES) & 1);
+        mbar_wait_nocall(&kv_full[st], (j / ATT_KV_STAGES) & 1);
         const uint32_t k_addr = smem_u32(kv_smem + st * 2 * ATT_K_BYTES);
         float s[32];
 #pragma unroll
diff --git a/omg_b200/csrc/gemm_tc.cu b/omg_b200/csrc/gemm_tc.cu
--- a/omg_b200/csrc/gemm_tc.cu
+++ b/omg_b200/csrc/gemm_tc.cu
@@ -26,7 +26,8 @@
     CUtensorMap b_maps[2];
     SegDev segs[OMG_MAX_SEGS];
     int n_segs;
-    int m_tiles, n_tiles;
+    int units;
+    int n_units;
     int tw, th, tiles_w, tiles_h;
     int img_w, img_h, img_b;
     int N, N_out;
@@ -39,6 +40,7 @@
     int residual_ld;
     int act_silu;
     float* stats_out;
+    int stats_unit_planes;
     const float* stats_in;
     int stats_parts;
     long long stats_rows;
@@ -56,22 +58,21 @@
     int cs_rb0, cs_rb_total;
 };
 
-template <int BN, int MT, bool CS>
+template <int UN, bool CS>
 struct GemmCfg {
-    static constexpr int WN = BN > 256 ? BN / 2 : BN;
-    static constexpr int NW = BN / WN;
-    static constexpr int ACC = MT * BN / 2;
-    static constexpr int A_BYTES = MT * BM * BK * 2;
-    static constexpr int B_BYTES = BN * BK * 2;
+    static constexpr int ACC = UN;
+    static constexpr int A_BYTES = BM * BK * 2;
+    static constexpr int B_BYTES = UN * BK * 2;
     static constexpr int STAGE_BYTES = A_BYTES + B_BYTES;
-    static constexpr int VEC_BYTES = 2 * MT * BN * 4;
-    static constexpr int CS_BYTES = CS ? 8 * MT * BN * 8 : 0;
+    static constexpr int VEC_BYTES = 2 * 2 * UN * 4;
+    static constexpr int CS_BYTES = CS ? 2 * 8 * (UN / 2) * 16 : 0;
     static constexpr int BARS_BYTES = 256;
     static constexpr int BUDGET = 227 * 1024 - 1024  - VEC_BYTES - CS_BYTES - BARS_BYTES;
     static constexpr int STAGES_RAW = BUDGET / STAGE_BYTES;
     static constexpr int STAGES = STAGES_RAW > 8 ? 8 : STAGES_RAW;
     static constexpr int SMEM_BYTES = 1024 + STAGES * STAGE_BYTES + VEC_BYTES + CS_BYTES + BARS_BYTES;
     static_assert(STAGES >= 2, "shared memory budget");
+    static_assert((2 * STAGES + 2) * 8 <= BARS_BYTES, "barrier space");
 };
 
 __device__ __forceinline__ float gelu_exact(float x) { return 0.5f * x * (1.0f + erff(x * 0.70710678118654752f)); }
@@ -81,35 +82,40 @@
     if constexpr (std::is_same_v<T, __nv_bfloat16>) {
         if constexpr (WN == 64) wgmma_ss_n64_bf16(*reinterpret_cast<float(*)[32]>(d), da, db, 1u);
         else if constexpr (WN == 128) wgmma_ss_n128_bf16(*reinterpret_cast<float(*)[64]>(d), da, db, 1u);
-        else if constexpr (WN == 160) wgmma_ss_n160_bf16(*reinterpret_cast<float(*)[80]>(d), da, db, 1u);
-        else wgmma_ss_n256_bf16(*reinterpret_cast<float(*)[128]>(d), da, db, 1u);
+        else wgmma_ss_n160_bf16(*reinterpret_cast<float(*)[80]>(d), da, db, 1u);
     } else {
         if constexpr (WN == 64) wgmma_ss_n64(*reinterpret_cast<float(*)[32]>(d), da, db, 1u);
         else if constexpr (WN == 128) wgmma_ss_n128(*reinterpret_cast<float(*)[64]>(d), da, db, 1u);
-        else if constexpr (WN == 160) wgmma_ss_n160(*reinterpret_cast<float(*)[80]>(d), da, db, 1u);
-        else wgmma_ss_n256(*reinterpret_cast<float(*)[128]>(d), da, db, 1u);
-    }
-}
-
-template <typename T, int BN, int EPI, int MT, int FEAT>
+        else wgmma_ss_n160(*reinterpret_cast<float(*)[80]>(d), da, db, 1u);
+    }
+}
+
+template <int STAGES>
+__device__ __forceinline__ void ring_advance(int& stage, uint32_t& phase, int n) {
+    stage += n;
+    const int wraps = stage / STAGES;
+    stage -= wraps * STAGES;
+    phase ^= (uint32_t)wraps & 1u;
+}
+
+template <typename T, int UN, int EPI, int FEAT>
 __global__ void __launch_bounds__(GEMM_THREADS, 1) gemm_tc_kernel(const __grid_constant__ GemmParams p) {
     using T2 = pair_t<T>;
     constexpr bool kStats = FEAT >= 1, kExtra = FEAT >= 2;
-    static_assert(EPI != OMG_EPI_GEGLU || (BN <= 256 && MT == 1), "GEGLU runs on single 128-row tiles");
-    using Cfg = GemmCfg<BN, MT, kStats>;
+    static_assert(EPI != OMG_EPI_GEGLU || UN == 160, "GEGLU runs on 160-wide units");
+    using Cfg = GemmCfg<UN, kStats>;
     constexpr int STAGES = Cfg::STAGES;
-    constexpr int NJ = BN / 8;
+    constexpr int NJ = UN / 8;
     extern __shared__ __align__(1024) uint8_t smem_raw[];
     uint8_t* smem = reinterpret_cast<uint8_t*>((reinterpret_cast<uintptr_t>(smem_raw) + 1023) & ~uintptr_t(1023));
-    float* s_bias = reinterpret_cast<float*>(smem + STAGES * Cfg::STAGE_BYTES);
-    float* s_c1 = s_bias + MT * BN;
-    float4* s_cs = reinterpret_cast<float4*>(s_c1 + MT * BN);
-    uint64_t* full_bar = reinterpret_cast<uint64_t*>(reinterpret_cast<uint8_t*>(s_cs) + Cfg::CS_BYTES);
+    float* s_vec = reinterpret_cast<float*>(smem + STAGES * Cfg::STAGE_BYTES);
+    float4* s_cs_all = reinterpret_cast<float4*>(s_vec + 2 * 2 * UN);
+    uint64_t* full_bar = reinterpret_cast<uint64_t*>(reinterpret_cast<uint8_t*>(s_cs_all) + Cfg::CS_BYTES);
     uint64_t* empty_bar = full_bar + STAGES;
+    uint64_t* turn_bar = empty_bar + STAGES;
 
     const int warp = threadIdx.x >> 5;
     const int lane = threadIdx.x & 31;
-    const int total_tiles = ((p.m_tiles + MT - 1) / MT) * p.n_tiles;
     const int tiles_per_img = p.tiles_w * p.tiles_h;
 
     if (warp == 8 && lane == 0) {
@@ -118,8 +124,10 @@
         tma_prefetch_desc(&p.b_maps[1]);
         for (int i = 0; i < STAGES; ++i) {
             mbar_init(&full_bar[i], 1);
-            mbar_init(&empty_bar[i], 2);
+            mbar_init(&empty_bar[i], 1);
         }
+        mbar_init(&turn_bar[0], 1);
+        mbar_init(&turn_bar[1], 1);
         fence_barrier_init();
     }
     __syncthreads();
@@ -131,14 +139,12 @@
         if (warp == 8 && lane == 0) {
             int stage = 0;
             uint32_t phase = 0;
-            for (int tile = blockIdx.x; tile < total_tiles; tile += gridDim.x) {
-                const int m_tile = (tile / p.n_tiles) * MT, n_tile = tile % p.n_tiles;
+            for (int u = blockIdx.x; u < p.units; u += gridDim.x) {
+                const int m_tile = u / p.n_units, nu = u % p.n_units;
                 const int b = m_tile / tiles_per_img;
                 const int rem = m_tile % tiles_per_img;
                 const int h0 = (rem / p.tiles_w) * p.th, w0 = (rem % p.tiles_w) * p.tw;
-                const int b1 = (m_tile + 1) / tiles_per_img, rem1 = (m_tile + 1) % tiles_per_img;
-                const int h1 = (rem1 / p.tiles_w) * p.th, w1 = (rem1 % p.tiles_w) * p.tw;
-                int n0 = n_tile * BN;
+                int n0 = nu * UN;
                 if (p.w_group_rows > 0) {
                     const long long tile_pix0 = ((long long)b * p.img_h + h0) * p.img_w + w0;
                     for (int g2 = 0; g2 + 1 < p.n_col_groups; ++g2)
@@ -147,18 +153,12 @@
                 for (int s = 0; s < p.n_segs; ++s) {
                     const SegDev sg = p.segs[s];
                     for (int kb = 0; kb < sg.k_blocks; ++kb) {
-                        mbar_wait(&empty_bar[stage], phase ^ 1);
+                        mbar_wait_nocall(&empty_bar[stage], phase ^ 1);
                         uint8_t* a_dst = smem + stage * Cfg::STAGE_BYTES;
                         uint8_t* b_dst = a_dst + Cfg::A_BYTES;
                         mbar_arrive_expect_tx(&full_bar[stage], Cfg::STAGE_BYTES);
                         tma_load_4d(a_dst, &p.a_maps[sg.a_map], &full_bar[stage], sg.a_c0 + kb * BK, w0 + sg.dx, h0 + sg.dy, b);
-                        if constexpr (MT == 2)
-                            tma_load_4d(a_dst + BM * BK * 2, &p.a_maps[sg.a_map], &full_bar[stage], sg.a_c0 + kb * BK,
-                                        w1 + sg.dx, h1 + sg.dy, b1);
-#pragma unroll
-                        for (int nw = 0; nw < Cfg::NW; ++nw)
-                            tma_load_2d(b_dst + nw * Cfg::WN * BK * 2, &p.b_maps[sg.b_map], &full_bar[stage],
-                                        sg.b_k0 + kb * BK, n0 + nw * Cfg::WN);
+                        tma_load_2d(b_dst, &p.b_maps[sg.b_map], &full_bar[stage], sg.b_k0 + kb * BK, n0);
                         if (++stage == STAGES) {
                             stage = 0;
                             phase ^= 1;
@@ -174,28 +174,36 @@
     const int wg = warp >> 2;
     const int wi = warp & 3;
     const int g = lane >> 2, c = lane & 3;
-    const int ctid = threadIdx.x;
+    const int wtid = threadIdx.x & 127;
+    float* s_bias = s_vec + wg * (2 * UN);
+    float* s_c1 = s_bias + UN;
+    float4* s_cs = s_cs_all + wg * (8 * (UN / 2));
+    int unit_kb = 0;
+    for (int s = 0; s < p.n_segs; ++s) unit_kb += p.segs[s].k_blocks;
     int stage = 0;
     uint32_t phase = 0;
+    if (wg == 1) ring_advance<STAGES>(stage, phase, unit_kb);
+    uint32_t turn_phase = wg == 0 ? 1u : 0u;
     float acc[Cfg::ACC];
 
-    for (int tile = blockIdx.x; tile < total_tiles; tile += gridDim.x) {
-        const int unit_m = (tile / p.n_tiles) * MT, n_tile = tile % p.n_tiles;
-        const int n0 = n_tile * BN;
+    for (int u = blockIdx.x + wg * gridDim.x; u < p.units; u += 2 * gridDim.x) {
+        const int m_tile = u / p.n_units, nu = u % p.n_units;
+        const int n0 = nu * UN;
+        const int b = m_tile / tiles_per_img;
+        const int rem = m_tile % tiles_per_img;
+        const int h0 = (rem / p.tiles_w) * p.th, w0 = (rem % p.tiles_w) * p.tw;
         const bool ln = p.stats_in != nullptr;
 
-        named_bar_sync(1, 256);
-        for (int sub = 0; sub < MT; ++sub) {
-            const int mt = unit_m + sub;
-            const int b = mt / tiles_per_img, rem = mt % tiles_per_img;
+        named_bar_sync(1 + wg, 128);
+        {
             size_t cg = 0;
             if (ln && p.n_col_groups > 1) {
-                const long long tile_pix0 = ((long long)b * p.img_h + (rem / p.tiles_w) * p.th) * p.img_w + (rem % p.tiles_w) * p.tw;
+                const long long tile_pix0 = ((long long)b * p.img_h + h0) * p.img_w + w0;
                 for (int g2 = 0; g2 + 1 < p.n_col_groups; ++g2)
                     if (tile_pix0 >= p.col_group_end[g2]) cg = g2 + 1;
                 cg *= (size_t)p.N;
             }
-            for (int j = ctid; j < BN; j += 256) {
+            for (int j = wtid; j < UN; j += 128) {
                 float v = 0.f, c1 = 0.f;
                 const int n = n0 + j;
                 if (n < p.N) {
@@ -207,37 +215,34 @@
                         if (p.rowvec && b < p.img_b) v += to_f32(static_cast<const T*>(p.rowvec)[(size_t)b * p.rowvec_ld + n]);
                     }
                 }
-                s_bias[sub * BN + j] = v;
-                s_c1[sub * BN + j] = c1;
+                s_bias[j] = v;
+                s_c1[j] = c1;
             }
         }
-        named_bar_sync(1, 256);
+        named_bar_sync(1 + wg, 128);
 
 #pragma unroll
         for (int i = 0; i < Cfg::ACC; ++i) acc[i] = 0.f;
+        mbar_wait_nocall(&turn_bar[wg], turn_phase);
+        turn_phase ^= 1;
         int prev_stage = -1;
         for (int s = 0; s < p.n_segs; ++s) {
             const int kbs = p.segs[s].k_blocks;
             for (int kb = 0; kb < kbs; ++kb) {
-                mbar_wait(&full_bar[stage], phase);
-                const uint32_t a_addr = smem_u32(smem + stage * Cfg::STAGE_BYTES) + (uint32_t)(wg * MT) * (64 * BK * 2);
-                const uint32_t b_addr = smem_u32(smem + stage * Cfg::STAGE_BYTES + Cfg::A_BYTES);
+                mbar_wait_nocall(&full_bar[stage], phase);
+                const uint32_t a_addr = smem_u32(smem + stage * Cfg::STAGE_BYTES);
+                const uint32_t b_addr = a_addr + Cfg::A_BYTES;
                 wgmma_fence();
 #pragma unroll
                 for (int k = 0; k < BK / 16; ++k) {
-#pragma unroll
-                    for (int i = 0; i < MT; ++i) {
-                        const uint64_t a_desc = gmma_desc_sw128(a_addr + i * (64 * BK * 2) + k * 32, 1024, 16);
-#pragma unroll
-                        for (int nw = 0; nw < Cfg::NW; ++nw) {
-                            const uint64_t b_desc = gmma_desc_sw128(b_addr + nw * (Cfg::WN * BK * 2) + k * 32, 1024, 16);
-                            wgmma_ss<T, Cfg::WN>(acc + i * (BN / 2) + nw * (Cfg::WN / 2), a_desc, b_desc);
-                        }
-                    }
+                    const uint64_t b_desc = gmma_desc_sw128(b_addr + k * 32, 1024, 16);
+#pragma unroll
+                    for (int i = 0; i < 2; ++i)
+                        wgmma_ss<T, UN>(acc + i * (UN / 2), gmma_desc_sw128(a_addr + i * (64 * BK * 2) + k * 32, 1024, 16), b_desc);
                 }
                 wgmma_commit();
                 wgmma_wait<1>();
-                if (prev_stage >= 0 && (ctid & 127) == 0) mbar_arrive(&empty_bar[prev_stage]);
+                if (prev_stage >= 0 && wtid == 0) mbar_arrive(&empty_bar[prev_stage]);
                 prev_stage = stage;
                 if (++stage == STAGES) {
                     stage = 0;
@@ -245,21 +250,15 @@
                 }
             }
         }
+        if (wtid == 0) mbar_arrive(&turn_bar[wg ^ 1]);
         wgmma_wait<0>();
         reg_fence(acc);
-        if ((ctid & 127) == 0) mbar_arrive(&empty_bar[prev_stage]);
-
-#pragma unroll
-        for (int i = 0; i < MT; ++i) {
-            const int blk = wg * MT + i;
-            const int sub = blk >> 1;
-            const int m_tile = unit_m + sub;
-            const int b = m_tile / tiles_per_img;
-            const int rem = m_tile % tiles_per_img;
-            const int h0 = (rem / p.tiles_w) * p.th, w0 = (rem % p.tiles_w) * p.tw;
-            const float* sb = s_bias + sub * BN;
-            const float* sc = s_c1 + sub * BN;
-            float* a = acc + i * (BN / 2);
+        if (wtid == 0) mbar_arrive(&empty_bar[prev_stage]);
+        ring_advance<STAGES>(stage, phase, unit_kb);
+
+#pragma unroll
+        for (int blk = 0; blk < 2; ++blk) {
+            float* a = acc + blk * (UN / 2);
             float row_sum[2] = {0.f, 0.f}, row_sq[2] = {0.f, 0.f};
             bool valid[2];
             size_t pix[2];
@@ -267,7 +266,7 @@
             float ln_a[2] = {1.f, 1.f}, ln_k[2] = {0.f, 0.f};
 #pragma unroll
             for (int h = 0; h < 2; ++h) {
-                const int et = (blk & 1) * 64 + wi * 16 + g + 8 * h;
+                const int et = blk * 64 + wi * 16 + g + 8 * h;
                 const int ph = h0 + et / p.tw, pw = w0 + et % p.tw;
                 valid[h] = (ph < p.img_h) && (pw < p.img_w) && (b < p.img_b);
                 pix[h] = ((size_t)b * p.img_h + ph) * p.img_w + pw;
@@ -284,7 +283,7 @@
                     ln_k[h] = -ln_a[h] * mu;
                 }
             }
-            float4* cs_slot = s_cs + (size_t)(blk * 4 + wi) * (BN / 2);
+            float4* cs_slot = s_cs + (size_t)(blk * 4 + wi) * (UN / 2);
 #pragma unroll
             for (int J = 0; J < NJ; ++J) {
                 const int col = 8 * J + 2 * c;
@@ -295,7 +294,7 @@
 #pragma unroll
                     for (int e = 0; e < 2; ++e) {
                         const float v = a[4 * J + 2 * h + e];
-                        x[h][e] = ln ? fmaf(ln_a[h], v, fmaf(ln_k[h], sc[col + e], sb[col + e])) : v + sb[col + e];
+                        x[h][e] = ln ? fmaf(ln_a[h], v, fmaf(ln_k[h], s_c1[col + e], s_bias[col + e])) : v + s_bias[col + e];
                     }
                 if constexpr (EPI == OMG_EPI_GEGLU) {
 #pragma unroll
@@ -376,7 +375,7 @@
             if constexpr (EPI != OMG_EPI_GEGLU) {
                 if (p.stats_out != nullptr) {
                     float2* so = reinterpret_cast<float2*>(p.stats_out);
-                    constexpr int PLANES = BN > 256 ? 4 : 2;
+                    const int kp = p.stats_unit_planes, plane0 = nu * kp;
 #pragma unroll
                     for (int h = 0; h < 2; ++h) {
                         float s = row_sum[h], q = row_sq[h];
@@ -385,25 +384,25 @@
                         s += __shfl_xor_sync(0xffffffffu, s, 2);
                         q += __shfl_xor_sync(0xffffffffu, q, 2);
                         if (c == 0 && valid[h]) {
-                            so[(size_t)(n_tile * PLANES) * p.stats_rows + pix[h]] = make_float2(s, q);
-                            for (int t = 1; t < PLANES; ++t) so[(size_t)(n_tile * PLANES + t) * p.stats_rows + pix[h]] = make_float2(0.f, 0.f);
+                            so[(size_t)plane0 * p.stats_rows + pix[h]] = make_float2(s, q);
+                            for (int t = 1; t < kp; ++t) so[(size_t)(plane0 + t) * p.stats_rows + pix[h]] = make_float2(0.f, 0.f);
                         }
                     }
                 }
             }
             if constexpr (EPI != OMG_EPI_GEGLU && kStats) {
                 if (p.col_stats != nullptr) {
-                    named_bar_sync(2 + wg * 2 + (wi >> 1), 64);
-                    const int q = (blk & 1) * 2 + (wi >> 1);
-                    const float4* s0 = s_cs + (size_t)(blk * 4 + (wi & 2)) * (BN / 2);
-                    const float4* s1 = s0 + BN / 2;
+                    named_bar_sync(3 + wg * 2 + (wi >> 1), 64);
+                    const int q = blk * 2 + (wi >> 1);
+                    const float4* s0 = s_cs + (size_t)(blk * 4 + (wi & 2)) * (UN / 2);
+                    const float4* s1 = s0 + UN / 2;
                     if (b < p.img_b) {
                         const size_t rb = (size_t)b * p.cs_rb_total + p.cs_rb0 + (size_t)rem * 4 + q;
-                        for (int cp = (wi & 1) * 32 + lane; cp < BN / 2; cp += 64) {
+                        for (int cp = (wi & 1) * 32 + lane; cp < UN / 2; cp += 64) {
                             const int col = n0 + 2 * cp;
                             if (col < p.N) {
-                                const float4 u = s0[cp], w = s1[cp];
-                                p.col_stats[(rb * p.N + col) >> 1] = make_float4(u.x + w.x, u.y + w.y, u.z + w.z, u.w + w.w);
+                                const float4 u4 = s0[cp], w4 = s1[cp];
+                                p.col_stats[(rb * p.N + col) >> 1] = make_float4(u4.x + w4.x, u4.y + w4.y, u4.z + w4.z, u4.w + w4.w);
                             }
                         }
                     }
@@ -421,33 +420,32 @@
     return make_tmap(m, dt, v.ptr, 4, dims, strides, box, sw);
 }
 
-template <typename T, int BN, int EPI, int MT, int FEAT>
+template <typename T, int UN, int EPI, int FEAT>
 static int launch_gemm_f(const GemmParams& p, cudaStream_t stream) {
-    using Cfg = GemmCfg<BN, MT, (FEAT >= 1)>;
+    using Cfg = GemmCfg<UN, (FEAT >= 1)>;
     static bool configured = false;
     static int num_sms = 0;
     if (!configured) {
-        OMG_CUDA(cudaFuncSetAttribute(gemm_tc_kernel<T, BN, EPI, MT, FEAT>, cudaFuncAttributeMaxDynamicSharedMemorySize,
+        OMG_CUDA(cudaFuncSetAttribute(gemm_tc_kernel<T, UN, EPI, FEAT>, cudaFuncAttributeMaxDynamicSharedMemorySize,
                                       Cfg::SMEM_BYTES));
         int dev = 0;
         OMG_CUDA(cudaGetDevice(&dev));
         OMG_CUDA(cudaDeviceGetAttribute(&num_sms, cudaDevAttrMultiProcessorCount, dev));
         configured = true;
     }
-    const int units = ((p.m_tiles + MT - 1) / MT) * p.n_tiles;
-    const int grid = std::min(units, num_sms);
-    OMG_CUDA(launch_pdl(gemm_tc_kernel<T, BN, EPI, MT, FEAT>, dim3(grid), dim3(GEMM_THREADS), Cfg::SMEM_BYTES, stream, p));
+    const int grid = std::min(p.units, num_sms);
+    OMG_CUDA(launch_pdl(gemm_tc_kernel<T, UN, EPI, FEAT>, dim3(grid), dim3(GEMM_THREADS), Cfg::SMEM_BYTES, stream, p));
     return check_launch("gemm_tc_kernel");
 }
 
-template <int BN, int EPI, int MT = 1>
+template <int UN, int EPI>
 static int launch_gemm(const GemmParams& p, cudaStream_t stream) {
     if constexpr (EPI == OMG_EPI_GEGLU) {
-        return launch_gemm_f<__half, BN, EPI, MT, 0>(p, stream);
+        return launch_gemm_f<__half, UN, EPI, 0>(p, stream);
     } else {
-        if (p.act_silu != 0 || p.residual_f32 != nullptr || p.out_f32 != nullptr) return launch_gemm_f<__half, BN, EPI, MT, 2>(p, stream);
-        if (p.col_stats != nullptr) return launch_gemm_f<__half, BN, EPI, MT, 1>(p, stream);
-        return launch_gemm_f<__half, BN, EPI, MT, 0>(p, stream);
+        if (p.act_silu != 0 || p.residual_f32 != nullptr || p.out_f32 != nullptr) return launch_gemm_f<__half, UN, EPI, 2>(p, stream);
+        if (p.col_stats != nullptr) return launch_gemm_f<__half, UN, EPI, 1>(p, stream);
+        return launch_gemm_f<__half, UN, EPI, 0>(p, stream);
     }
 }
 
@@ -457,28 +455,21 @@
     return (double)((tiles + PLAN_SMS - 1) / PLAN_SMS) * (cols + TILE_OVERHEAD);
 }
 
-static bool use_tall_tiles(long m_tiles, long n_tiles, long k_blocks) {
-    if (m_tiles < 2 || k_blocks < 16) return false;
-    return tile_time(((m_tiles + 1) / 2) * n_tiles, 320.0) < tile_time(m_tiles * n_tiles, 160.0);
-}
-
 constexpr long K_PLAN_LONG = 1000;
-static int pick_block_n(int N, int epilogue, long m_tiles, long k_plan, long k_blocks, bool* prefer_tall) {
-    if (prefer_tall) *prefer_tall = false;
+static int pick_block_n(int N, int epilogue, long m_tiles, long k_plan) {
     if (epilogue == OMG_EPI_GEGLU) return 256;
     const int cands[5] = {256, 160, 128, 64, 160};
     int best = 256;
     double best_t = 1e30;
     for (int i = 0; i < 5; ++i) {
-        const bool tall = i == 4;
-        if (tall && (k_plan < 16 || m_tiles < 2)) continue;
+        const bool pair = i == 4;
+        if (pair && (k_plan < 16 || m_tiles < 2)) continue;
         const long nt = (N + cands[i] - 1) / cands[i];
-        const long mt = tall ? (m_tiles + 1) / 2 : m_tiles;
-        const double t = tile_time(nt * mt, tall ? 2.0 * cands[i] : cands[i]);
+        const long mt = pair ? (m_tiles + 1) / 2 : m_tiles;
+        const double t = tile_time(nt * mt, pair ? 2.0 * cands[i] : cands[i]);
         if (t < best_t - 1e-9) {
             best_t = t;
             best = cands[i];
-            if (prefer_tall) *prefer_tall = tall && k_blocks >= 16;
         }
     }
     return best;
@@ -494,7 +485,7 @@
     while (tw / 2 >= W && tw > 1) tw /= 2;
     const int th = 128 / tw;
     const long m_tiles = (long)((W + tw - 1) / tw) * ((H + th - 1) / th) * B;
-    const int bn = pick_block_n(N, epilogue, m_tiles, K_PLAN_LONG, 0, nullptr);
+    const int bn = pick_block_n(N, epilogue, m_tiles, K_PLAN_LONG);
     if (block_n) *block_n = bn;
     if (n_tiles) *n_tiles = 2 * ((N + bn - 1) / bn);
     return 0;
@@ -556,20 +547,22 @@
     p.img_w = W;
     p.img_h = H;
     p.img_b = B;
-    p.m_tiles = p.tiles_w * p.tiles_h * B;
+    const int m_tiles = p.tiles_w * p.tiles_h * B;
     p.N = d->N;
     p.N_out = N_out;
-    bool prefer_tall = false;
     const long k_blocks_hint = (long)(d->Ktot + (d->w2 ? d->K2tot : 0)) / 64;
     int bn = d->block_n ? d->block_n
-                        : pick_block_n(d->N, d->epilogue, p.m_tiles, d->row_stats_out ? K_PLAN_LONG : k_blocks_hint,
-                                       k_blocks_hint, &prefer_tall);
+                        : pick_block_n(d->N, d->epilogue, m_tiles, d->row_stats_out ? K_PLAN_LONG : k_blocks_hint);
     OMG_CHECK(bn == 64 || bn == 128 || bn == 160 || bn == 256 || bn == 320, "omg_gemm: block_n=%d unsupported", bn);
     OMG_CHECK(bn != 320 || (!geglu && d->N % 320 == 0), "omg_gemm: block_n=320 needs N %% 320 == 0 and no GEGLU");
     OMG_CHECK(d->cta_pair == 0 || d->cta_pair == 1 || d->cta_pair == 3, "omg_gemm: cta_pair=%d unsupported (0, 1 or 3)",
               d->cta_pair);
     if (geglu) bn = 256;
-    p.n_tiles = (d->N + bn - 1) / bn;
+    const int unit_n = geglu ? 160 : (bn > 160 ? bn / 2 : bn);
+    const int tile_units = geglu ? 1 : bn / unit_n;
+    p.n_units = geglu ? (d->N + 159) / 160 : (d->N + bn - 1) / bn * tile_units;
+    p.units = m_tiles * p.n_units;
+    p.stats_unit_planes = (bn == 320 ? 4 : 2) / tile_units;
     p.bias = d->bias;
     p.rowvec = d->rowvec;
     p.rowvec_ld = d->rowvec_ld;
@@ -632,7 +625,7 @@
         const uint64_t planes = d->w_group_planes > 0 ? (uint64_t)d->w_group_planes : 1;
         const uint64_t dims[2] = {(uint64_t)d->Ktot, (uint64_t)d->N * planes};
         const uint64_t strides[2] = {1, (uint64_t)d->Ktot};
-        const uint32_t box[2] = {BK, (uint32_t)(bn > 256 ? bn / 2 : bn)};
+        const uint32_t box[2] = {BK, (uint32_t)unit_n};
         if (make_tmap(&p.b_maps[0], tdt, d->w, 2, dims, strides, box, CU_TENSOR_MAP_SWIZZLE_128B)) return 1;
         p.b_maps[1] = p.b_maps[0];
     }
@@ -640,7 +633,7 @@
         OMG_CHECK(d->K2tot >= 8 && d->K2tot % 8 == 0, "omg_gemm: K2tot=%d must be a positive multiple of 8", d->K2tot);
         const uint64_t dims[2] = {(uint64_t)d->K2tot, (uint64_t)d->N};
         const uint64_t strides[2] = {1, (uint64_t)d->K2tot};
-        const uint32_t box[2] = {BK, (uint32_t)(bn > 256 ? bn / 2 : bn)};
+        const uint32_t box[2] = {BK, (uint32_t)unit_n};
         if (make_tmap(&p.b_maps[1], tdt, d->w2, 2, dims, strides, box, CU_TENSOR_MAP_SWIZZLE_128B)) return 1;
     }
     OMG_CHECK(d->d.sw % 2 == 0 && d->d.sh % 2 == 0 && d->d.sb % 2 == 0 && (reinterpret_cast<uintptr_t>(d->d.ptr) & 3) == 0,
@@ -665,33 +658,18 @@
         p.segs[s] = SegDev{sg.a_idx, sg.dx, sg.dy, sg.a_c0, (sg.k_len + BK - 1) / BK, sg.b_k0, sg.b_idx};
     }
 
-    long k_blocks = 0;
-    for (int i = 0; i < p.n_segs; ++i) k_blocks += p.segs[i].k_blocks;
-    bool pair_ok = true;
-    for (int i = 0; i + 1 < p.n_col_groups; ++i)
-        pair_ok = pair_ok && (H > 1 ? (p.col_group_end[i] / img_pix * p.tiles_w * p.tiles_h) % 2 == 0
-                                    : p.col_group_end[i] % 256 == 0);
-    const bool tall = bn == 160 && !geglu && pair_ok &&
-                      (d->cta_pair == 3 ||
-                       (d->cta_pair == 0 && (prefer_tall || use_tall_tiles(p.m_tiles, p.n_tiles, k_blocks))));
     if (bf16) {
-        if (tall) return launch_gemm_f<__nv_bfloat16, 160, OMG_EPI_NONE, 2, 0>(p, stream);
-        switch (bn) {
-            case 64: return launch_gemm_f<__nv_bfloat16, 64, OMG_EPI_NONE, 1, 0>(p, stream);
-            case 128: return launch_gemm_f<__nv_bfloat16, 128, OMG_EPI_NONE, 1, 0>(p, stream);
-            case 160: return launch_gemm_f<__nv_bfloat16, 160, OMG_EPI_NONE, 1, 0>(p, stream);
-            case 320: return launch_gemm_f<__nv_bfloat16, 320, OMG_EPI_NONE, 1, 0>(p, stream);
-            default: return launch_gemm_f<__nv_bfloat16, 256, OMG_EPI_NONE, 1, 0>(p, stream);
+        switch (unit_n) {
+            case 64: return launch_gemm_f<__nv_bfloat16, 64, OMG_EPI_NONE, 0>(p, stream);
+            case 128: return launch_gemm_f<__nv_bfloat16, 128, OMG_EPI_NONE, 0>(p, stream);
+            default: return launch_gemm_f<__nv_bfloat16, 160, OMG_EPI_NONE, 0>(p, stream);
         }
     }
-    if (bn == 320) return launch_gemm<320, OMG_EPI_NONE>(p, stream);
-    if (tall) return launch_gemm<160, OMG_EPI_NONE, 2>(p, stream);
-    if (geglu) return launch_gemm<256, OMG_EPI_GEGLU>(p, stream);
-    switch (bn) {
+    if (geglu) return launch_gemm<160, OMG_EPI_GEGLU>(p, stream);
+    switch (unit_n) {
         case 64: return launch_gemm<64, OMG_EPI_NONE>(p, stream);
         case 128: return launch_gemm<128, OMG_EPI_NONE>(p, stream);
-        case 160: return launch_gemm<160, OMG_EPI_NONE>(p, stream);
-        default: return launch_gemm<256, OMG_EPI_NONE>(p, stream);
+        default: return launch_gemm<160, OMG_EPI_NONE>(p, stream);
     }
 }
 
diff --git a/omg_b200/csrc/ptx.cuh b/omg_b200/csrc/ptx.cuh
--- a/omg_b200/csrc/ptx.cuh
+++ b/omg_b200/csrc/ptx.cuh
@@ -81,6 +81,14 @@
             __trap();
         }
     }
+}
+
+__device__ __forceinline__ void mbar_wait_nocall(uint64_t* bar, uint32_t parity) {
+    if (mbar_try_wait(bar, parity)) return;
+    const long long t0 = clock64();
+    uint32_t spins = 0;
+    while (!mbar_try_wait_long(bar, parity))
+        if ((++spins & 0x3FF) == 0 && clock64() - t0 > OMG_MBAR_TIMEOUT_CYCLES) __trap();
 }
 
 __device__ __forceinline__ float fast_exp2(float x) {
```

New measurement: 0.1960 (median of 6 runs). +3.7%, better.
